# nihaomiao/WACV23_TSNet

Measured on AMD Instinct MI355X. Metric: retargeted frames/sec at bs=4, 256x256, n_source=3; max-abs delta vs ref, higher is better.
Workload: dtype f32 (convolutions: fp16 x 2 split of the scaled fp32 operands, 3 exact MFMA products, two-level fp32 accumulate; fp32-class accuracy); 1 GPU; TSNet(label_nc=2,n_blocks=0,n_downsampling=3,n_source=3) forward, fp32, B=4 per GPU, 256x256 (BASELINE.json configs[1]); global_batch=4, parallelism=replicas x1 (batch-sharded, weights broadcast once)

## Files before the change

### include/tsnet_abi.h

```cpp
#ifndef TSNET_ABI_H
#define TSNET_ABI_H

#include <stddef.h>
#include <stdint.h>

#ifdef __cplusplus
extern "C" {
#endif

#define TSNET_ABI_VERSION 5
#define TSNET_MAX_SOURCES 8

enum {
    TSNET_OK = 0,
    TSNET_ERR_ARG = -1,
    TSNET_ERR_WEIGHT = -2,
    TSNET_ERR_HIP = -3,
    TSNET_ERR_NOMEM = -4
};

typedef struct tsnet_engine* tsnet_handle;

typedef struct tsnet_cfg {
    int label_nc;
    int n_blocks;
    int n_downsampling;
    int n_source;
    int ngf;
    int enc_blocks;
    int addcoords;
    int pose_composite;
    float pose_mean[3];
    int height, width;
    int max_batch;
    int operand_mode;
} tsnet_cfg;

#define TSNET_NPROD_F16 16

int tsnet_abi_version(void);
int tsnet_create(const tsnet_cfg* cfg, tsnet_handle* out);
int tsnet_load_weights(tsnet_handle h, const char* name, const float* data, const int64_t* shape, int rank);
int tsnet_finalize(tsnet_handle h, void* stream);
void tsnet_destroy(tsnet_handle h);
const char* tsnet_last_error(tsnet_handle h);

int tsnet_num_params(tsnet_handle h);
int tsnet_param_info(tsnet_handle h, int index, const char** name, int64_t shape_out[4], int* rank);

int tsnet_packed_weights(tsnet_handle h, void** dev_ptr, size_t* bytes);

int tsnet_forward(tsnet_handle h,
                  const float* const* src_img, const float* const* src_lbl, const float* const* src_bbox,
                  const float* tar_lbl, const float* tar_bbox,
                  float* out_rgb, float* out_flow, int B, void* stream);

int tsnet_set_source_divisors(tsnet_handle h, const float* div, int n);

int tsnet_set_sources(tsnet_handle h, const float* const* src_img, const float* const* src_lbl,
                      const float* const* src_bbox, int B, void* stream);
int tsnet_forward_target(tsnet_handle h, const float* tar_lbl, const float* tar_bbox,
                         float* out_rgb, float* out_flow, int B, void* stream);

int tsnet_set_sources_shared(tsnet_handle h, const float* const* src_img, const float* const* src_lbl,
                             const float* const* src_bbox, void* stream);

int tsnet_bank_capacity(tsnet_handle h);
int tsnet_bank_put(tsnet_handle h, int first_slot, int count, const float* const* src_img, const float* const* src_lbl,
                   const float* const* src_bbox, const float* div, void* stream);
int tsnet_forward_bank(tsnet_handle h, const int* slots, int Kc, const float* tar_lbl, const float* tar_bbox,
                       float* out_rgb, float* out_flow, int B, void* stream);

int tsnet_forward_u8(tsnet_handle h, const uint8_t* const* src_img, const uint8_t* const* src_lbl, const uint8_t* const* src_bbox,
                     const uint8_t* tar_lbl, const uint8_t* tar_bbox, const float* mean_bgr,
                     float* out_rgb, float* out_flow, int B, void* stream);
int tsnet_set_sources_u8(tsnet_handle h, const uint8_t* const* src_img, const uint8_t* const* src_lbl, const uint8_t* const* src_bbox,
                         const float* mean_bgr, int B, int shared, void* stream);
int tsnet_forward_target_u8(tsnet_handle h, const uint8_t* tar_lbl, const uint8_t* tar_bbox,
                            float* out_rgb, float* out_flow, int B, void* stream);
int tsnet_bank_put_u8(tsnet_handle h, int first_slot, int count, const uint8_t* const* src_img, const uint8_t* const* src_lbl,
                      const uint8_t* const* src_bbox, const float* mean_bgr, const float* div, void* stream);
int tsnet_forward_bank_u8(tsnet_handle h, const int* slots, int Kc, const uint8_t* tar_lbl, const uint8_t* tar_bbox,
                          float* out_rgb, float* out_flow, int B, void* stream);

int tsnet_train_extras(tsnet_handle h, const float* const* src_img, const float* tar_img, int B,
                       float* warp_src_img, float* losses, void* stream);

int tsnet_stage_ptr(tsnet_handle h, const char* name, const float** dev_ptr, size_t* count);

double tsnet_forward_macs(tsnet_handle h, int B);

#define TSNET_TIMING_CLASSES 9
enum { TSNET_T_CONV = 0, TSNET_T_STATS = 1, TSNET_T_ELEMWISE = 2, TSNET_T_FLOW = 3, TSNET_T_WARP = 4,
       TSNET_T_PACK = 5, TSNET_T_UPSAMPLE = 6, TSNET_T_OTHER = 7,
       TSNET_T_CONV_RES = 8  };
int tsnet_timing_enable(tsnet_handle h, int on);
int tsnet_timing_read(tsnet_handle h, double ms_out[TSNET_TIMING_CLASSES], int64_t launches_out[TSNET_TIMING_CLASSES], int reset);

int tsnet_op_conv2d(const float* x, int N, int H, int W, int Cin,
                    const float* w_oihw, const float* bias, int Cout, int ksize, int stride, int pad, int pad_mode,
                    const float* in_alpha, const float* in_beta, int in_relu, float bound, int nprod, int kernel, int tile,
                    float* y, void* stream);
int tsnet_op_conv2d_cat(const float* x, const float* x2, int N, int H, int W, int C1, int C2, int x2_nmod,
                        const float* w_oihw, const float* bias, int Cout, int ksize, int stride, int pad, int pad_mode,
                        float bound, int nprod, float* y, void* stream);
int tsnet_op_head(const float* x, int N, int H, int W, int C, const float* in_alpha, const float* in_beta,
                  const float* w_oihw, const float* bias, int composite, const float* bg, float* y, void* stream);
int tsnet_op_instnorm_stats(const float* x, int N, int HW, int C, float* alpha, float* beta, void* stream);
int tsnet_op_norm_act(const float* x, const float* alpha, const float* beta, int relu, const float* resid,
                      int N, int HW, int C, float* y, void* stream);
int tsnet_op_upsample2x(const float* x, const float* alpha, const float* beta, int relu,
                        int N, int H, int W, int C, float* y, void* stream);
int tsnet_op_flow(const float* tar_fea, const float* src_fea, const float* tar_bbox, const float* src_bbox,
                  int B, int h, int w, int C, int H, int W, float* flow, void* stream);
int tsnet_op_flow_k(const float* tar_fea, const float* src_fea, const float* tar_bbox, const float* src_bbox,
                    int B, int K, int h, int w, int C, int H, int W, float* flow, int variant, int repeat, float* ms_out, void* stream);
int tsnet_flow_plan(int B, int h, int w, int C);
int tsnet_op_warp(const float* src_fea, const float* flow, int B, int h, int w, int C, float* out, void* stream);
int tsnet_op_warp_k(const float* src_fea, const float* flow, int B, int K, int h, int w, int C, float* out, int repeat, float* ms_out, void* stream);
int tsnet_op_warp_k_shared(const float* src_fea, const float* flow, int B, int K, int SB, int h, int w, int C, float* out, void* stream);
int tsnet_op_add_stats(const float* x, const float* add, int add_nmod, int x_sb, int N, int HW, int C,
                       float* y, float* alpha, float* beta, void* stream);
int tsnet_op_finalize_stats(const double* part, int N, int S, int C, int HW, float* alpha, float* beta, void* stream);
int tsnet_op_fuse_tail(const float* src_fea, const float* tar_fea, const float* y2, const float* alpha, const float* beta,
                       int B, int K, int SB, int P, int C1, float* zbar, void* stream);
int tsnet_op_flow_k_slots(const float* tar_fea, const float* src_fea, const float* tar_bbox, const float* src_bbox,
                          int B, int K, int h, int w, int C, int H, int W, float* flow, int variant, int repeat, float* ms_out,
                          const int* slots, int n_src, void* stream);
int tsnet_op_warp_k_slots(const float* src_fea, const float* flow, int B, int K, int h, int w, int C, float* out,
                          const int* slots, int n_src, void* stream);
int tsnet_op_add_stats_slots(const float* x, const float* add, int add_nmod, int N, int HW, int C,
                             float* y, float* alpha, float* beta, const int* slots, int n_src, void* stream);
int tsnet_op_fuse_tail_slots(const float* src_fea, const float* tar_fea, const float* y2, const float* alpha, const float* beta,
                             int B, int K, int P, int C1, float* zbar, const int* slots, int n_src, void* stream);
int tsnet_op_pack_input(const float* const* img, const float* const* lbl, int S, int B, int H, int W, int L, int nimg, int Cp, int coords,
                        const float* img_div, float* out, unsigned int* amax, void* stream);
int tsnet_op_pack_input_u8(const uint8_t* const* img, const uint8_t* const* lbl, const uint8_t* const* bbox, int S, int B, int H, int W, int L,
                           int nimg, int Cp, int coords, const float* img_div, const float* mean_bgr, float* out, float* bbox_out,
                           unsigned int* amax, void* stream);
int tsnet_op_upsample2x_st(const float* x, const float* alpha, const float* beta, int relu,
                           int N, int H, int W, int C, int x_bf16, int y_bf16, float* y, void* stream);
const char* tsnet_op_last_error(void);

int tsnet_frame_stats(const float* x, int B, int C, int HW, float div, float* mean, float* std_unbiased, void* stream);
int tsnet_demo_postprocess(const float* rec, int B, int H, int W, const float* gen_mean, const float* gen_std,
                           const float* ref_mean, const float* ref_std, const float* img_mean_over_255,
                           unsigned char* out_rgb, void* stream);

int tsnet_fit_face_curves(const double* keypoints, int F, double* curves);
int tsnet_raster_face(const double* keypoints, const double* curves, int F, int h, int w, int bw, unsigned char* edges, unsigned char* bbox, void* stream);
int tsnet_vl2ch(const float* labels, int B, int HW, int num_classes, float* out, void* stream);

int tsnet_face_adapt_stats(const double* kp, int F, double* stats);
int tsnet_face_adapt_apply(const double* stats, double* kp, int F);
int tsnet_smooth_keypoints(const double* in, int F, int P, double* out);

int tsnet_resize_label(const unsigned char* in, int F, int h, int w, int OH, int OW, const double* wts_rows, int lw_rows,
                       const double* wts_cols, int lw_cols, float* out, void* stream);
int tsnet_fit_pose_curves(const double* pts, int F, int flags, double* curves);
int tsnet_raster_pose(const double* pts, const double* curves, int F, int h, int w, int win_x0, int win_y0, int win_x1, int win_y1, int flags,
                      unsigned char* labels, void* stream);
int tsnet_label_bbox(const unsigned char* labels, int F, int h, int w, unsigned char* bbox, void* stream);
int tsnet_resize_pad(const unsigned char* in, int F, int h, int w, const int* ytab, const int* xtab, int oh, int ow,
                     int pad_top, int pad_left, int OH, int OW, int binarise, float* out, void* stream);

int tsnet_bench_conv(int N, int H, int W, int Cin, int Cout, int ksize, int stride, int pad, int pad_mode, int norm,
                     int variant, int iters, float* ms_out, void* stream);

void tsnet_debug_counters(int64_t out[4], int reset);

void tsnet_linspace(int n, float* out);
void tsnet_coord_table(int H, int W, float* out);

int tsnet_bicubic_taps(int n_in, int n_out);
int tsnet_bicubic_table(int n_in, int n_out, int* first, int* count, int* coef);
int tsnet_prepare_frames(const unsigned char* frames, int F, int h, int w, int x0, int y0, int x1, int y1,
                         const int* xfirst, const int* xcount, const int* xcoef, int xtaps,
                         const int* yfirst, const int* ycount, const int* ycoef, int ytaps,
                         int oh, int ow, int pad_top, int pad_left, int OH, int OW, const float* mean_bgr, float* out, void* stream);
int tsnet_prepare_frames_u8(const unsigned char* frames, int F, int h, int w, int x0, int y0, int x1, int y1,
                            const int* xfirst, const int* xcount, const int* xcoef, int xtaps,
                            const int* yfirst, const int* ycount, const int* ycoef, int ytaps,
                            int oh, int ow, int pad_top, int pad_left, int OH, int OW, unsigned char* out, void* stream);

int tsnet_paste_frames(const unsigned char* gen, const unsigned char* mask, int F, int GH, int GW, int sx0, int sy0, int sx1, int sy1,
// ... 26 lines not shown
```

### wacv23_tsnet_amd/_lib.py

```python
from __future__ import annotations

import ctypes as C
import os

import torch

_HERE = os.path.dirname(os.path.abspath(__file__))
LIB_PATH = os.path.join(_HERE, "lib", "libtsnet_hip.so")
MAX_SOURCES = 8
TIMING_CLASSES = 9
TIMING_NAMES = ("conv", "stats", "elementwise", "flow", "warp", "pack", "upsample", "other", "conv_res")

ABI_SYMBOLS = (
    "tsnet_abi_version", "tsnet_create", "tsnet_load_weights", "tsnet_finalize", "tsnet_destroy",
    "tsnet_last_error", "tsnet_num_params", "tsnet_param_info", "tsnet_packed_weights",
    "tsnet_forward", "tsnet_set_source_divisors", "tsnet_set_sources", "tsnet_set_sources_shared", "tsnet_forward_target", "tsnet_train_extras", "tsnet_stage_ptr",
    "tsnet_forward_macs", "tsnet_timing_enable", "tsnet_timing_read",
    "tsnet_op_conv2d", "tsnet_op_conv2d_cat", "tsnet_op_head", "tsnet_op_instnorm_stats", "tsnet_op_norm_act", "tsnet_op_upsample2x",
    "tsnet_op_flow", "tsnet_op_flow_k", "tsnet_flow_plan", "tsnet_op_warp", "tsnet_op_warp_k", "tsnet_op_warp_k_shared", "tsnet_op_add_stats", "tsnet_op_finalize_stats", "tsnet_op_fuse_tail", "tsnet_op_pack_input", "tsnet_op_upsample2x_st", "tsnet_op_last_error", "tsnet_frame_stats", "tsnet_demo_postprocess", "tsnet_fit_face_curves", "tsnet_raster_face", "tsnet_vl2ch", "tsnet_fit_pose_curves", "tsnet_raster_pose", "tsnet_label_bbox", "tsnet_resize_pad", "tsnet_resize_label", "tsnet_bench_conv", "tsnet_debug_counters", "tsnet_linspace", "tsnet_coord_table",
    "tsnet_bicubic_taps", "tsnet_bicubic_table", "tsnet_prepare_frames",
    "tsnet_face_adapt_stats", "tsnet_face_adapt_apply", "tsnet_smooth_keypoints",
    "tsnet_bank_capacity", "tsnet_bank_put", "tsnet_forward_bank",
    "tsnet_op_flow_k_slots", "tsnet_op_warp_k_slots", "tsnet_op_add_stats_slots", "tsnet_op_fuse_tail_slots",
    "tsnet_forward_u8", "tsnet_set_sources_u8", "tsnet_forward_target_u8", "tsnet_bank_put_u8", "tsnet_forward_bank_u8",
    "tsnet_op_pack_input_u8", "tsnet_prepare_frames_u8",
    "tsnet_paste_frames",
    "tsnet_prepare_frames_boxes", "tsnet_prepare_frames_boxes_u8", "tsnet_paste_frames_boxes",
    "tsnet_face_labels_boxes", "tsnet_face_labels_boxes_u8",
)


class TsnetCfg(C.Structure):
    _fields_ = [
        ("label_nc", C.c_int), ("n_blocks", C.c_int), ("n_downsampling", C.c_int), ("n_source", C.c_int),
        ("ngf", C.c_int), ("enc_blocks", C.c_int), ("addcoords", C.c_int), ("pose_composite", C.c_int),
        ("pose_mean", C.c_float * 3), ("height", C.c_int), ("width", C.c_int), ("max_batch", C.c_int), ("operand_mode", C.c_int),
    ]


_fp = C.POINTER(C.c_float)
_vp = C.c_void_p


def bind(lib: C.CDLL) -> C.CDLL:
    lib.tsnet_abi_version.restype = C.c_int
    lib.tsnet_create.argtypes = [C.POINTER(TsnetCfg), C.POINTER(_vp)]
    lib.tsnet_load_weights.argtypes = [_vp, C.c_char_p, _vp, C.POINTER(C.c_int64), C.c_int]
    lib.tsnet_finalize.argtypes = [_vp, _vp]
    lib.tsnet_destroy.argtypes = [_vp]
    lib.tsnet_destroy.restype = None
    lib.tsnet_last_error.argtypes = [_vp]
    lib.tsnet_last_error.restype = C.c_char_p
    lib.tsnet_num_params.argtypes = [_vp]
    lib.tsnet_param_info.argtypes = [_vp, C.c_int, C.POINTER(C.c_char_p), C.POINTER(C.c_int64), C.POINTER(C.c_int)]
    lib.tsnet_packed_weights.argtypes = [_vp, C.POINTER(_vp), C.POINTER(C.c_size_t)]
    pp = C.POINTER(_vp)
    lib.tsnet_forward.argtypes = [_vp, pp, pp, pp, _vp, _vp, _vp, _vp, C.c_int, _vp]
    lib.tsnet_set_source_divisors.argtypes = [_vp, _fp, C.c_int]
    lib.tsnet_set_sources.argtypes = [_vp, pp, pp, pp, C.c_int, _vp]
    if hasattr(lib, "tsnet_set_sources_shared"):
        lib.tsnet_set_sources_shared.argtypes = [_vp, pp, pp, pp, _vp]
    lib.tsnet_forward_target.argtypes = [_vp, _vp, _vp, _vp, _vp, C.c_int, _vp]
    lib.tsnet_train_extras.argtypes = [_vp, pp, _vp, C.c_int, _vp, _vp, _vp]
    lib.tsnet_stage_ptr.argtypes = [_vp, C.c_char_p, C.POINTER(_vp), C.POINTER(C.c_size_t)]
    lib.tsnet_forward_macs.argtypes = [_vp, C.c_int]
    lib.tsnet_forward_macs.restype = C.c_double
    lib.tsnet_timing_enable.argtypes = [_vp, C.c_int]
    lib.tsnet_timing_read.argtypes = [_vp, C.POINTER(C.c_double), C.POINTER(C.c_int64), C.c_int]
    lib.tsnet_op_conv2d.argtypes = [_vp, C.c_int, C.c_int, C.c_int, C.c_int, _vp, _vp, C.c_int, C.c_int, C.c_int,
                                    C.c_int, C.c_int, _vp, _vp, C.c_int, C.c_float, C.c_int, C.c_int, C.c_int, _vp, _vp]
    lib.tsnet_op_conv2d_cat.argtypes = [_vp, _vp] + [C.c_int] * 6 + [_vp, _vp] + [C.c_int] * 5 + [C.c_float, C.c_int, _vp, _vp]
    lib.tsnet_op_head.argtypes = [_vp, C.c_int, C.c_int, C.c_int, C.c_int, _vp, _vp, _vp, _vp, C.c_int, _fp, _vp, _vp]
    lib.tsnet_op_instnorm_stats.argtypes = [_vp, C.c_int, C.c_int, C.c_int, _vp, _vp, _vp]
    lib.tsnet_op_norm_act.argtypes = [_vp, _vp, _vp, C.c_int, _vp, C.c_int, C.c_int, C.c_int, _vp, _vp]
    lib.tsnet_op_upsample2x.argtypes = [_vp, _vp, _vp, C.c_int, C.c_int, C.c_int, C.c_int, C.c_int, _vp, _vp]
    lib.tsnet_resize_label.argtypes = [_vp, C.c_int, C.c_int, C.c_int, C.c_int, C.c_int, _vp, C.c_int, _vp, C.c_int, _vp, _vp]
    lib.tsnet_op_flow.argtypes = [_vp, _vp, _vp, _vp, C.c_int, C.c_int, C.c_int, C.c_int, C.c_int, C.c_int, _vp, _vp]
    lib.tsnet_op_flow_k.argtypes = [_vp, _vp, _vp, _vp] + [C.c_int] * 7 + [_vp, C.c_int, C.c_int, _fp, _vp]
    lib.tsnet_flow_plan.argtypes = [C.c_int] * 4
    lib.tsnet_op_warp.argtypes = [_vp, _vp, C.c_int, C.c_int, C.c_int, C.c_int, _vp, _vp]
    if hasattr(lib, "tsnet_op_warp_k"):
        lib.tsnet_op_warp_k.argtypes = [_vp, _vp] + [C.c_int] * 5 + [_vp, C.c_int, _fp, _vp]
    if hasattr(lib, "tsnet_op_fuse_tail"):
        lib.tsnet_op_warp_k_shared.argtypes = [_vp, _vp] + [C.c_int] * 6 + [_vp, _vp]
        lib.tsnet_op_add_stats.argtypes = [_vp, _vp] + [C.c_int] * 5 + [_vp, _vp, _vp, _vp]
        lib.tsnet_op_finalize_stats.argtypes = [_vp] + [C.c_int] * 4 + [_vp, _vp, _vp]
        lib.tsnet_op_fuse_tail.argtypes = [_vp] * 5 + [C.c_int] * 5 + [_vp, _vp]
        lib.tsnet_op_pack_input.argtypes = [pp, pp] + [C.c_int] * 8 + [_fp, _vp, _vp, _vp]
        lib.tsnet_op_upsample2x_st.argtypes = [_vp, _vp, _vp] + [C.c_int] * 7 + [_vp, _vp]
    lib.tsnet_op_last_error.restype = C.c_char_p
    lib.tsnet_frame_stats.argtypes = [_vp, C.c_int, C.c_int, C.c_int, C.c_float, _vp, _vp, _vp]
    lib.tsnet_demo_postprocess.argtypes = [_vp, C.c_int, C.c_int, C.c_int, _vp, _vp, _vp, _vp, _fp, _vp, _vp]
    lib.tsnet_fit_face_curves.argtypes = [_vp, C.c_int, _vp]
    lib.tsnet_fit_pose_curves.argtypes = [_vp, C.c_int, C.c_int, _vp]
    lib.tsnet_raster_face.argtypes = [_vp, _vp, C.c_int, C.c_int, C.c_int, C.c_int, _vp, _vp, _vp]
    lib.tsnet_vl2ch.argtypes = [_vp, C.c_int, C.c_int, C.c_int, _vp, _vp]
    lib.tsnet_raster_pose.argtypes = [_vp, _vp] + [C.c_int] * 8 + [_vp, _vp]
    lib.tsnet_label_bbox.argtypes = [_vp, C.c_int, C.c_int, C.c_int, _vp, _vp]
    lib.tsnet_resize_pad.argtypes = [_vp, C.c_int, C.c_int, C.c_int, _vp, _vp] + [C.c_int] * 7 + [_vp, _vp]
    lib.tsnet_bench_conv.argtypes = [C.c_int] * 12 + [_fp, _vp]
    lib.tsnet_debug_counters.argtypes = [C.POINTER(C.c_int64), C.c_int]
    lib.tsnet_debug_counters.restype = None
    lib.tsnet_linspace.argtypes = [C.c_int, _fp]
    lib.tsnet_linspace.restype = None
    lib.tsnet_coord_table.argtypes = [C.c_int, C.c_int, _fp]
    lib.tsnet_coord_table.restype = None
    if hasattr(lib, "tsnet_prepare_frames"):
        lib.tsnet_bicubic_taps.argtypes = [C.c_int, C.c_int]
        lib.tsnet_bicubic_table.argtypes = [C.c_int, C.c_int, _vp, _vp, _vp]
        lib.tsnet_prepare_frames.argtypes = [_vp] + [C.c_int] * 7 + [_vp, _vp, _vp, C.c_int, _vp, _vp, _vp, C.c_int] + [C.c_int] * 6 + [_fp, _vp, _vp]
    if hasattr(lib, "tsnet_face_adapt_stats"):
        lib.tsnet_face_adapt_stats.argtypes = [_vp, C.c_int, _vp]
        lib.tsnet_face_adapt_apply.argtypes = [_vp, _vp, C.c_int]
        lib.tsnet_smooth_keypoints.argtypes = [_vp, C.c_int, C.c_int, _vp]
    if hasattr(lib, "tsnet_forward_bank"):
        _ip = C.POINTER(C.c_int)
        lib.tsnet_bank_capacity.argtypes = [_vp]
        lib.tsnet_bank_put.argtypes = [_vp, C.c_int, C.c_int, pp, pp, pp, _fp, _vp]
        lib.tsnet_forward_bank.argtypes = [_vp, _ip, C.c_int, _vp, _vp, _vp, _vp, C.c_int, _vp]
        lib.tsnet_op_flow_k_slots.argtypes = [_vp, _vp, _vp, _vp] + [C.c_int] * 7 + [_vp, C.c_int, C.c_int, _fp, _ip, C.c_int, _vp]
        lib.tsnet_op_warp_k_slots.argtypes = [_vp, _vp] + [C.c_int] * 5 + [_vp, _ip, C.c_int, _vp]
        lib.tsnet_op_add_stats_slots.argtypes = [_vp, _vp] + [C.c_int] * 4 + [_vp, _vp, _vp, _ip, C.c_int, _vp]
        lib.tsnet_op_fuse_tail_slots.argtypes = [_vp] * 5 + [C.c_int] * 4 + [_vp, _ip, C.c_int, _vp]
    if hasattr(lib, "tsnet_forward_u8"):
        _ip = C.POINTER(C.c_int)
        lib.tsnet_forward_u8.argtypes = [_vp, pp, pp, pp, _vp, _vp, _fp, _vp, _vp, C.c_int, _vp]
        lib.tsnet_set_sources_u8.argtypes = [_vp, pp, pp, pp, _fp, C.c_int, C.c_int, _vp]
        lib.tsnet_forward_target_u8.argtypes = [_vp, _vp, _vp, _vp, _vp, C.c_int, _vp]
        lib.tsnet_bank_put_u8.argtypes = [_vp, C.c_int, C.c_int, pp, pp, pp, _fp, _fp, _vp]
        lib.tsnet_forward_bank_u8.argtypes = [_vp, _ip, C.c_int, _vp, _vp, _vp, _vp, C.c_int, _vp]
        lib.tsnet_op_pack_input_u8.argtypes = [pp, pp, pp] + [C.c_int] * 8 + [_fp, _fp, _vp, _vp, _vp, _vp]
        lib.tsnet_prepare_frames_u8.argtypes = [_vp] + [C.c_int] * 7 + [_vp, _vp, _vp, C.c_int, _vp, _vp, _vp, C.c_int] + [C.c_int] * 6 + [_vp, _vp]
    if hasattr(lib, "tsnet_paste_frames"):
        lib.tsnet_paste_frames.argtypes = [_vp, _vp] + [C.c_int] * 7 + [_vp, _vp, _vp, C.c_int, _vp, _vp, _vp, C.c_int] + [_vp] + [C.c_int] * 6 + [_vp]
    if hasattr(lib, "tsnet_paste_frames_boxes"):
        lib.tsnet_prepare_frames_boxes.argtypes = [_vp] + [C.c_int] * 3 + [_vp, _vp, _vp, C.c_int] + [C.c_int] * 6 + [_fp, _vp, _vp]
        lib.tsnet_prepare_frames_boxes_u8.argtypes = [_vp] + [C.c_int] * 3 + [_vp, _vp, _vp, C.c_int] + [C.c_int] * 6 + [_vp, _vp]
        lib.tsnet_paste_frames_boxes.argtypes = [_vp, _vp] + [C.c_int] * 7 + [_vp, _vp, _vp, C.c_int] + [_vp, C.c_int, C.c_int, _vp]
    if hasattr(lib, "tsnet_face_labels_boxes"):
        for fn in (lib.tsnet_face_labels_boxes, lib.tsnet_face_labels_boxes_u8):
            fn.argtypes = [_vp, _vp, C.c_int, _vp, _vp, _vp, C.c_int, C.c_int, _vp, C.c_longlong, C.c_int, C.c_int, _vp, _vp, _vp]
    return lib


_cached = None


def load_tools() -> C.CDLL:
    from . import build as _b
    if not os.path.exists(_b.OUT_TOOLS):
        raise RuntimeError(f"{_b.OUT_TOOLS} is missing: run `python -m wacv23_tsnet_amd.build --tools`")
    return bind(C.CDLL(_b.OUT_TOOLS))


def load() -> C.CDLL:
    global _cached
    if _cached is not None:
        return _cached
    if not os.path.exists(LIB_PATH):
        raise RuntimeError(
            f"{LIB_PATH} is missing: the HIP extension is not built. Run "
            "`python -c 'import __graft_entry__ as g; g.build()'` (needs hipcc). "
            "There is no CPU fallback for the TS-Net forward path.")
    try:
        _cached = bind(C.CDLL(LIB_PATH))
    except OSError as e:
        raise RuntimeError(f"failed to load {LIB_PATH}: {e}") from e
    if _cached.tsnet_abi_version() != 5:
        raise RuntimeError("libtsnet_hip.so ABI version mismatch; rebuild")
    return _cached
```

### wacv23_tsnet_amd/csrc/conv_common.hpp

```cpp
#pragma once
#include <hip/hip_runtime.h>

namespace tsnet {

typedef float f32x16 __attribute__((ext_vector_type(16)));
struct alignas(16) F4 { float v[4]; };

constexpr unsigned kOOB = 0x80000000u;
constexpr int kPatchCols = 32;
constexpr int kPatchRows = 4;

constexpr int kNprodF16 = 16;
constexpr bool one_product(int nprod) { return nprod == 1 || nprod == kNprodF16; }

#ifndef TSNET_BUF_LOAD16
typedef __amdgpu_buffer_rsrc_t tsnet_brsrc_t;
__device__ __forceinline__ tsnet_brsrc_t tsnet_make_brsrc(const void* p, unsigned bytes) {
    return __builtin_amdgcn_make_buffer_rsrc(const_cast<void*>(p), 0, (int)bytes, 0x00020000);
}
#define TSNET_BUF_LOAD16(rsrc, voff, soff) __builtin_bit_cast(F4, __builtin_amdgcn_raw_buffer_load_b128((rsrc), (int)(voff), (int)(soff), 0))
#endif
#ifndef TSNET_BUF_LOAD8
struct alignas(8) F2 { float v[2]; };
#define TSNET_BUF_LOAD8(rsrc, voff, soff) __builtin_bit_cast(F2, __builtin_amdgcn_raw_buffer_load_b64((rsrc), (int)(voff), (int)(soff), 0))
// ... 142 lines not shown
    int xcd_gn;
    float* fin_alpha; float* fin_beta; int* fin_counter; int fin_S; float fin_eps;
    unsigned* amax_out;
    int x_bf16, y_bf16;
    int w1_chunk, w1_tab2;
};

__device__ __forceinline__ void bf16x8_widen(const F4& p, F4 (&o)[2]) {
#pragma unroll
    for (int e = 0; e < 4; ++e) {
        const unsigned w = __builtin_bit_cast(unsigned, p.v[e]);
        o[e >> 1].v[(e & 1) * 2] = __builtin_bit_cast(float, w << 16);
        o[e >> 1].v[(e & 1) * 2 + 1] = __builtin_bit_cast(float, w & 0xFFFF0000u);
    }
}

__device__ __forceinline__ void load_x_octet(const tsnet_brsrc_t& rs, bool xb16, unsigned voff, unsigned soff, F4 (&o)[2]) {
    if (xb16) {
        const F4 p = TSNET_BUF_LOAD16(rs, voff >> 1, soff >> 1);
        bf16x8_widen(p, o);
    } else {
        o[0] = TSNET_BUF_LOAD16(rs, voff, soff);
        o[1] = TSNET_BUF_LOAD16(rs, voff, soff + 16u);
    }
}

__device__ __forceinline__ void h2_device_scale(const unsigned* amax, float add, float& scale, float& unscale) {
    const float bound = __builtin_bit_cast(float, __hip_atomic_load(amax, __ATOMIC_RELAXED, __HIP_MEMORY_SCOPE_AGENT)) + add;
    int e = 0;
    (void)frexpf(bound, &e);
    int sa = 15 - e;
    sa = sa > 24 ? 24 : (sa < -24 ? -24 : sa);
    scale = ldexpf(1.0f, sa);
    unscale = ldexpf(1.0f, -sa);
}

__device__ __forceinline__ void split_h2(float v, unsigned& hi, unsigned& lo) {
    const _Float16 h = (_Float16)v;
    const _Float16 l = (_Float16)(v - (float)h);
    hi = (unsigned)__builtin_bit_cast(unsigned short, h);
    lo = (unsigned)__builtin_bit_cast(unsigned short, l);
}

__device__ __forceinline__ void split_h2_octet(const F4& x0, const F4& x1, F4& H, F4& L) {
    unsigned hw[4], lw[4];
    TSNET_SPLIT_2PAIRS(x0.v[0], x0.v[1], x0.v[2], x0.v[3], hw[0], lw[0], hw[1], lw[1]);
    TSNET_SPLIT_2PAIRS(x1.v[0], x1.v[1], x1.v[2], x1.v[3], hw[2], lw[2], hw[3], lw[3]);
#pragma unroll
    for (int e = 0; e < 4; ++e) { H.v[e] = __builtin_bit_cast(float, hw[e]); L.v[e] = __builtin_bit_cast(float, lw[e]); }
}

template <bool F16 = false>
__device__ __forceinline__ void one_plane_octet(const F4& x0, const F4& x1, F4& H) {
    unsigned hw[4];
#pragma unroll
    for (int e = 0; e < 2; ++e) {
        hw[e] = cvt_pk_one<F16>(x0.v[2 * e], x0.v[2 * e + 1]);
        hw[2 + e] = cvt_pk_one<F16>(x1.v[2 * e], x1.v[2 * e + 1]);
    }
#pragma unroll
    for (int e = 0; e < 4; ++e) H.v[e] = __builtin_bit_cast(float, hw[e]);
}

template <bool AFFINE, bool KEEP = true>
__device__ __forceinline__ void transform_octet(const F4 (&sx)[2], const float* ta, int Cin, float in_scale, float relu_floor, float keep, F4 (&t)[2]) {
    if (AFFINE) {
#pragma unroll
        for (int q = 0; q < 2; ++q) {
            const F4 al = *reinterpret_cast<const F4*>(ta + q * 4), be = *reinterpret_cast<const F4*>(ta + Cin + q * 4);
#pragma unroll
            for (int e = 0; e < 4; ++e) {
                const float v = __builtin_fmaxf(__builtin_fmaf(sx[q].v[e], al.v[e], be.v[e]), relu_floor);
                t[q].v[e] = KEEP ? v * keep : v;
            }
        }
    } else {
#pragma unroll
        for (int q = 0; q < 2; ++q)
#pragma unroll
            for (int e = 0; e < 4; ++e) t[q].v[e] = __builtin_fmaxf(sx[q].v[e] * in_scale, relu_floor);
    }
}

template <int BN, int WARPS_M, int WARPS_N, int MT, int NTL, int STAT_WAVE = 0, typename MOf>
__device__ __forceinline__ void conv_epilogue(const ConvArgs& a, f32x16 (&tot)[MT][NTL], unsigned char* smem_raw, int tid, int wave, int n0,
                                              size_t stat_tile, MOf m_of, const bool active = true) {
    constexpr int WM = MT * 32, WN = NTL * 32;
    const int lane = tid & 63, li = lane & 31, lh = lane >> 5;
    const int wm0 = (wave / WARPS_N) * WM, wn0 = (wave % WARPS_N) * WN;
    const int hw = a.Ho * a.Wo;
    double csum[NTL], csq[NTL];
#pragma unroll
    for (int j = 0; j < NTL; ++j) { csum[j] = 0.0; csq[j] = 0.0; }
    float vmax = 0.f;
#pragma unroll
    for (int i = 0; i < MT; ++i) {
#pragma unroll
        for (int j = 0; j < NTL; ++j) {
            const int n = n0 + wn0 + j * 32 + li;
            const bool nok = n < a.Cout;
            const float bv = (a.bias && nok) ? a.bias[n] : 0.f;
#pragma unroll
            for (int r = 0; r < 16; ++r) {
                const int m = m_of(wm0 + i * 32 + (r & 3) + 8 * (r >> 2) + 4 * lh);
                const bool mok = active && m >= 0;
                float v = tot[i][j][r] + bv;
                if (a.addend && nok && mok) {
                    const int img = m / hw;
                    v += a.addend[((size_t)(img % a.add_nmod) * hw + (m - img * hw)) * a.Cout + n];
                }
                tot[i][j][r] = v;
                if (a.stat_part && mok) { csum[j] += (double)v; csq[j] += (double)v * (double)v; }
                if (nok && mok) vmax = __builtin_fmaxf(vmax, __builtin_fabsf(v));
            }
        }
    }
    if (a.amax_out) tsnet_publish_amax(a.amax_out + stat_tile / (size_t)a.tpi, vmax);
    if (a.stat_part) {
        __syncthreads();
        double* red = reinterpret_cast<double*>(smem_raw);
#pragma unroll
        for (int j = 0; j < NTL; ++j) {
            const double s2 = csum[j] + __shfl_xor(csum[j], 32);
            const double q2 = csq[j] + __shfl_xor(csq[j], 32);
            if (lh == 0 && active) {
                double* o = red + ((size_t)(wave / WARPS_N) * BN + wn0 + j * 32 + li) * 2;
                o[0] = s2; o[1] = q2;
            }
        }
        __syncthreads();
        const int stid = tid - 64 * STAT_WAVE;
        if (stid >= 0 && stid < BN && n0 + stid < a.Cout) {
            double s = 0.0, q = 0.0;
#pragma unroll
            for (int wmi = 0; wmi < WARPS_M; ++wmi) { s += red[((size_t)wmi * BN + stid) * 2]; q += red[((size_t)wmi * BN + stid) * 2 + 1]; }
            double* o = a.stat_part + (stat_tile * a.Cout + n0 + stid) * 2;
            if (a.fin_counter) {
                __hip_atomic_store(o, s, __ATOMIC_RELAXED, __HIP_MEMORY_SCOPE_AGENT);
                __hip_atomic_store(o + 1, q, __ATOMIC_RELAXED, __HIP_MEMORY_SCOPE_AGENT);
            } else {
                o[0] = s; o[1] = q;
            }
        }
        if (a.fin_counter) {
            const int S = a.fin_S;
            const int img = (int)(stat_tile / (size_t)S);
            const int ntn = (a.Npad + 31) / 32;
            int* counter = a.fin_counter + (size_t)img * ntn + n0 / 32;
            const bool mine = stid >= 0 && stid < BN && n0 + stid < a.Cout;
            auto fold = [&](const double* p0, int cnt, size_t step, double& sm, double& sq) __attribute__((always_inline)) {
                double gs[4] = {0, 0, 0, 0}, gq[4] = {0, 0, 0, 0};
                for (int t0 = 0; t0 < cnt; t0 += 8) {
                    double v[8], w[8];
#pragma unroll
                    for (int u = 0; u < 8; ++u) {
                        const double* p = p0 + (size_t)(t0 + u < cnt ? t0 + u : cnt - 1) * step;
                        v[u] = __hip_atomic_load(p, __ATOMIC_RELAXED, __HIP_MEMORY_SCOPE_AGENT);
                        w[u] = __hip_atomic_load(p + 1, __ATOMIC_RELAXED, __HIP_MEMORY_SCOPE_AGENT);
                    }
#pragma unroll
                    for (int u = 0; u < 8; ++u) {
                        const bool in = t0 + u < cnt;
                        gs[u & 3] += in ? v[u] : 0.0;
                        gq[u & 3] += in ? w[u] : 0.0;
                    }
                }
// ... 65 lines not shown
```

### wacv23_tsnet_amd/csrc/conv_h2.hpp

```cpp
#pragma once
#include "conv_common.hpp"

namespace tsnet {

template <int PR, int BN, int WARPS_M, int WARPS_N, int NPROD, bool AFFINE, int HABL = 0, int OPT = 0>
__device__ __forceinline__ void h2_tile(const ConvArgs& a, unsigned char* smem_raw, const int tile_m, const int n0) {
    constexpr int BM = PR * kPatchCols;
    constexpr int NW = WARPS_M * WARPS_N;
    static_assert(NW == 4, "four waves: patch blocks are dealt w, w+4");
    static_assert(one_product(NPROD) || NPROD == 3 || NPROD == 4, "one (a bf16 or an fp16 plane), three or four products");
    constexpr bool ONEP = one_product(NPROD), F16P = NPROD == kNprodF16;
    constexpr int NPL = ONEP ? 1 : 2;
    constexpr bool DEEP = (OPT & 8) != 0;
    constexpr int BD = DEEP ? 9 : ((OPT & 32) ? 6 : 3);
    constexpr bool ONE_LEVEL = ONEP;
    constexpr bool ZPAD_KEEP = (OPT & 1) != 0;
    constexpr int CH = (OPT & 2) ? 1 : ((OPT & 4) ? 4 : 2);
    constexpr int KG = (OPT & 16) ? 2 : 1;
    constexpr int WM = BM / WARPS_M, WN = BN / WARPS_N;
    constexpr int MT = WM / 32, NTL = WN / 32;
    static_assert(WARPS_M * MT == PR, "a wave covers MT whole patch rows");
    constexpr int NRW = MT + 2;
    constexpr int PC = kPatchCols + 2, PP = (PR + 2) * PC;
    constexpr int PBLK = (PP + 31) / 32;
    static_assert(PBLK <= 8, "two staging rounds");
    constexpr int REGION = PBLK * 512;
    constexpr int PLANE_P = 2 * REGION, PATCH_BYTES = NPL * PLANE_P;
    constexpr int OFF_SINK = 2 * 2 * PLANE_P;
    constexpr int GROUP_BYTES = OFF_SINK + 2048;
    constexpr int OFF_TAB = KG * GROUP_BYTES;

    const int tid = threadIdx.x;
    const int lane = tid & 63;
    const int wave_all = TSNET_UNIFORM(tid >> 6);
    const int kg = KG == 1 ? 0 : wave_all >> 2;
    const int wave = KG == 1 ? wave_all : (wave_all & 3);
    unsigned char* const gbase = smem_raw + kg * GROUP_BYTES;
    const int wrow = wave / WARPS_N;
    const int wn0 = (wave % WARPS_N) * WN;
    const int li = lane & 31, lh = lane >> 5;

    const int tcols = a.Wo / kPatchCols, tper = (a.Ho / PR) * tcols;
    const int img = tile_m / tper, tin = tile_m - img * tper;
    const int oy0 = (tin / tcols) * PR, ox0 = (tin % tcols) * kPatchCols;
    const int ncc = a.Cin >> 4;
    float in_scale = a.in_scale, in_unscale = a.in_unscale;
    if (NPROD != 1 && a.in_amax) h2_device_scale(a.in_amax + img, a.in_bound_add, in_scale, in_unscale);

    const size_t planew = (size_t)((a.nchunks + 1) / 2 * 2) * a.Npad * 16;
    const bool xb16 = NPROD == 1 && a.x_bf16;
    const tsnet_brsrc_t rsx = tsnet_make_brsrc(a.x, (unsigned)((size_t)a.N * a.H * a.W * a.Cin * (xb16 ? 2 : 4)));
    tsnet_brsrc_t rsw[NPL];
#pragma unroll
    for (int p = 0; p < NPL; ++p) rsw[p] = tsnet_make_brsrc(a.w + p * planew, (unsigned)(planew * 2));

    const int oct = lane >> 5;
    unsigned vP[2];
    float vM[2];
#pragma unroll
    for (int r = 0; r < 2; ++r) {
        const int pp = (wave + 4 * r) * 32 + (lane & 31);
        const int pr = pp / PC, pc = pp - pr * PC;
        int iy = oy0 - 1 + pr, ix = ox0 - 1 + pc;
        bool ok = pp < PP;
        if (a.reflect) {
            iy = iy < 0 ? -iy : iy;
            iy = iy >= a.H ? 2 * (a.H - 1) - iy : iy;
            ix = ix < 0 ? -ix : ix;
            ix = ix >= a.W ? 2 * (a.W - 1) - ix : ix;
        } else {
            ok = ok && iy >= 0 && iy < a.H && ix >= 0 && ix < a.W;
        }
        const int pix = iy * a.W + ix;
        vP[r] = ok ? (unsigned)(((img * a.H * a.W + pix) * a.Cin + oct * 8) * 4) : kOOB;
        vM[r] = ok ? 1.f : 0.f;
    }
    float* tab = reinterpret_cast<float*>(smem_raw + OFF_TAB);
    if (AFFINE) {
        for (int c = tid; c < a.Cin; c += 256 * KG) {
            tab[c] = a.in_alpha[(size_t)img * a.Cin + c] * in_scale;
            tab[a.Cin + c] = a.in_beta[(size_t)img * a.Cin + c] * in_scale;
        }
        __syncthreads();
    }
    const float relu_floor = a.in_relu ? 0.f : -__builtin_inff();
    auto slab_of = [&](int lc) __attribute__((always_inline)) { return lc * KG + kg; };
    F4 sx[2][2];
    auto stage_load_x = [&](int cn, int r) __attribute__((always_inline)) {
        if (NPROD == 1) load_x_octet(rsx, xb16, vP[r], (unsigned)(slab_of(cn) * 64), sx[r]);
        else {
#pragma unroll
            for (int q = 0; q < 2; ++q) sx[r][q] = TSNET_BUF_LOAD16(rsx, vP[r], (unsigned)(slab_of(cn) * 64 + q * 16));
        }
    };
    auto stage_store = [&](int cn, int par, int r) __attribute__((always_inline)) {
        const int b = wave + 4 * r;
        F4 t[2];
        const float* ta = tab + (slab_of(cn) < ncc ? slab_of(cn) * 16 : 0) + oct * 8;
        transform_octet<AFFINE, ZPAD_KEEP>(sx[r], ta, a.Cin, in_scale, relu_floor, vM[r], t);
        unsigned char* dst = gbase + (b < PBLK ? par * PATCH_BYTES + oct * REGION + b * 512 : OFF_SINK + oct * 512) + (lane & 31) * 16;
        F4 Hh, Ll;
        if (ONEP) {
            one_plane_octet<F16P>(t[0], t[1], Hh);
            *reinterpret_cast<F4*>(dst) = Hh;
        } else {
            split_h2_octet(t[0], t[1], Hh, Ll);
            *reinterpret_cast<F4*>(dst) = Hh;
            *reinterpret_cast<F4*>(dst + (b < PBLK ? PLANE_P : 1024)) = Ll;
        }
    };

    const unsigned vB = (unsigned)((wn0 + li) * 32 + (lh ^ ((li >> 3) & 1)) * 16);
    constexpr bool DB = MT > 2;
    static_assert(!DB || NRW == 6, "the double-buffered form fetches two rows of the next tap column per step");
    F4 ar[DB ? 2 : 1][NRW][NPL], bf[BD][NPL][NTL];
    auto tap_of = [](int s) __attribute__((always_inline)) { return (s % 3) * 3 + s / 3; };
    const int wB = a.Npad * 32, wT = ncc * wB;
    int wsl = slab_of(0) * wB + n0 * 32;
    auto load_b = [&](int set, int dslab, int s) __attribute__((always_inline)) {
        const int soff = wsl + dslab * KG * wB + tap_of(s) * wT;
#pragma unroll
        for (int p = 0; p < NPL; ++p)
#pragma unroll
            for (int j = 0; j < NTL; ++j) bf[set][p][j] = TSNET_BUF_LOAD16(rsw[p], vB + j * 1024u, (unsigned)soff);
    };
    const unsigned char* abase = gbase + lh * REGION + (wrow * MT * PC + li) * 16;
    auto load_row = [&](int r, int par, int kx) __attribute__((always_inline)) {
        const unsigned char* pbase = abase + par * PATCH_BYTES;
#pragma unroll
        for (int p = 0; p < NPL; ++p) ar[DB ? (kx & 1) : 0][r][p] = *reinterpret_cast<const F4*>(pbase + p * PLANE_P + (r * PC + kx) * 16);
    };

    f32x16 acc[MT][NTL], tot[MT][NTL];
#pragma unroll
    for (int i = 0; i < MT; ++i)
#pragma unroll
        for (int j = 0; j < NTL; ++j)
#pragma unroll
            for (int r = 0; r < 16; ++r) { acc[i][j][r] = 0.f; tot[i][j][r] = 0.f; }

    auto product = [&](int kx, int ky, int sb, int pa, int pb, bool fresh) __attribute__((always_inline)) {
#pragma unroll
        for (int i = 0; i < MT; ++i)
#pragma unroll
            for (int j = 0; j < NTL; ++j) {
                f32x16 c = acc[i][j];
                if (fresh) {
#pragma unroll
                    for (int r = 0; r < 16; ++r) c[r] = 0.f;
                }
                if (NPROD == 1) acc[i][j] = TSNET_MFMA_BF16(ar[DB ? (kx & 1) : 0][i + ky][pa], bf[sb][pb][j], c);
                else acc[i][j] = TSNET_MFMA_F16(ar[DB ? (kx & 1) : 0][i + ky][pa], bf[sb][pb][j], c);
            }
    };
    auto step = [&](int cc, int par, int s, bool first, bool last) __attribute__((always_inline)) {
        const int kx = s / 3, ky = s % 3;
        const bool fresh = !ONE_LEVEL && first;
        const int s2 = (s + BD - 1) % 9;
        if (!(HABL & 2)) load_b((par * 9 + s + BD - 1) % BD, s + BD - 1 >= 9 ? 1 : 0, s2);
        if (!(HABL & 4)) {
            if (DB) {
                if (kx < 2) { load_row(2 * ky, par, kx + 1); load_row(2 * ky + 1, par, kx + 1); }
            } else {
                if (ky < 2) load_row(ky + MT, par, kx);
                if (kx < 2 && ky == 1) {
#pragma unroll
                    for (int r = 0; r + 1 < MT; ++r) load_row(r, par, kx + 1);
                }
                if (kx < 2 && ky == 2) load_row(MT - 1, par, kx + 1);
            }
        }
        if (s == 0 && !(HABL & 1)) stage_load_x(cc + 1, 0);
        if (s == (DEEP ? 1 : 3) && !(HABL & 1)) stage_load_x(cc + 1, 1);
        const int SB = (par * 9 + s) % BD;
        if (ONEP) {
            product(kx, ky, SB, 0, 0, fresh);
        } else {
            if (NPROD == 4) product(kx, ky, SB, NPL - 1, NPL - 1, fresh);
            product(kx, ky, SB, NPL - 1, 0, fresh && NPROD == 3);
            product(kx, ky, SB, 0, NPL - 1, false);
            product(kx, ky, SB, 0, 0, false);
        }
        if (s == (DEEP ? 5 : 2) && !(HABL & 1)) stage_store(cc + 1, par ^ 1, 0);
        if (s == (DEEP ? 7 : 5) && !(HABL & 1)) stage_store(cc + 1, par ^ 1, 1);
        __builtin_amdgcn_sched_barrier(0);
        if (!ONE_LEVEL && last && !(HABL & 8)) {
#pragma unroll
            for (int i = 0; i < MT; ++i)
#pragma unroll
                for (int j = 0; j < NTL; ++j)
#pragma unroll
                    for (int r = 0; r < 16; ++r) tot[i][j][r] += acc[i][j][r];
        }
    };
    auto slab = [&](int cc, int par, bool open, bool close) __attribute__((always_inline)) {
        if (!(HABL & 16)) __syncthreads();
        if ((!(HABL & 4) || cc == 0) && !(DB && (HABL & 8) && cc > 0)) {
#pragma unroll
            for (int r = 0; r < (DB ? NRW : MT); ++r) load_row(r, par, 0);
        }
#pragma unroll
        for (int s = 0; s < 9; ++s) step(cc, par, s, open && s == 0, close && s == 8);
        wsl += KG * wB;
    };

    stage_load_x(0, 0); stage_load_x(0, 1);
#pragma unroll
    for (int i = 0; i < BD - 1; ++i) load_b(i, 0, i);
    stage_store(0, 0, 0); stage_store(0, 0, 1);
    if (HABL & 2) load_b(2, 0, 2);
    if (HABL & 4) {
        __syncthreads();
#pragma unroll
        for (int r = 0; r < NRW; ++r) load_row(r, 0, 0);
    }
    const int nloc = ncc / KG;
    int cc = 0;
    if (CH == 4) {
        for (; cc + 4 <= nloc; cc += 4) { slab(cc, 0, true, false); slab(cc + 1, 1, false, false); slab(cc + 2, 0, false, false); slab(cc + 3, 1, false, true); }
    }
    if (CH == 1) {
        for (; cc + 2 <= nloc; cc += 2) { slab(cc, 0, true, true); slab(cc + 1, 1, true, true); }
    } else {
        for (; cc + 2 <= nloc; cc += 2) { slab(cc, 0, true, false); slab(cc + 1, 1, false, true); }
    }
    if (cc < nloc) slab(cc, 0, true, true);
    if (ONE_LEVEL) {
#pragma unroll
        for (int i = 0; i < MT; ++i)
#pragma unroll
            for (int j = 0; j < NTL; ++j) tot[i][j] = acc[i][j];
    }
    if (KG == 2) {
        __syncthreads();
        float* fold = reinterpret_cast<float*>(smem_raw) + (size_t)wave * (MT * NTL * 16 * 64) + lane;
        if (kg == 1) {
#pragma unroll
            for (int i = 0; i < MT; ++i)
#pragma unroll
                for (int j = 0; j < NTL; ++j)
#pragma unroll
                    for (int r = 0; r < 16; ++r) fold[((i * NTL + j) * 16 + r) * 64] = tot[i][j][r];
        }
        __syncthreads();
        if (kg == 0) {
#pragma unroll
            for (int i = 0; i < MT; ++i)
#pragma unroll
                for (int j = 0; j < NTL; ++j)
#pragma unroll
                    for (int r = 0; r < 16; ++r) tot[i][j][r] += fold[((i * NTL + j) * 16 + r) * 64];
        }
    }

    const float unscale = a.w_unscale ? in_unscale * a.w_unscale[0] : in_unscale;
#pragma unroll
    for (int i = 0; i < MT; ++i)
#pragma unroll
        for (int j = 0; j < NTL; ++j)
#pragma unroll
            for (int r = 0; r < 16; ++r) tot[i][j][r] *= unscale;
    const int m_img = img * a.Ho * a.Wo;
    conv_epilogue<BN, WARPS_M, WARPS_N, MT, NTL>(a, tot, smem_raw, tid, wave, n0, (size_t)img * tper + tin,
                                                 [&](int l) { return m_img + (oy0 + (l >> 5)) * a.Wo + ox0 + (l & 31); }, kg == 0);
}

constexpr int h2_lds_bytes(int PR, int Cin, int KG = 1) { return KG * (2 * 2 * 2 * (((PR + 2) * (kPatchCols + 2) + 31) / 32) * 512 + 2048) + 2 * Cin * 4; }

template <int PR, int BN, int WARPS_M, int WARPS_N, int NPROD, int OPT>
constexpr int h2_wgs_per_cu() { return (OPT & 16) ? 1 : ((BN / WARPS_N) * (PR / WARPS_M) * ((OPT & 8) ? 2 : 1) <= (one_product(NPROD) ? 128 : 64) ? ((OPT & 64) ? 4 : 3) : 2); }

template <int PR, int BN, int WARPS_M, int WARPS_N, int NPROD, bool AFFINE, int HABL = 0, int OPT = 0>
__global__ __launch_bounds__((OPT & 16) ? 512 : 256, (h2_wgs_per_cu<PR, BN, WARPS_M, WARPS_N, NPROD, OPT>()))
void conv_h2_kernel(ConvArgs a) {
    HIP_DYNAMIC_SHARED(__attribute__((aligned(16))) unsigned char, smem_raw)
    int tile_m, tile_n;
    tile_of_block(blockIdx.x, a.tiles_m, a.tiles_n, a.xcd_gn, tile_m, tile_n);
    h2_tile<PR, BN, WARPS_M, WARPS_N, NPROD, AFFINE, HABL, OPT>(a, smem_raw, tile_m, tile_n * BN);
}

template <int NPROD>
__device__ __forceinline__ void h2s_tile(const ConvArgs& a, unsigned char* smem_raw, const int tile_m, const int n0) {
    constexpr int BN = 64, WARPS_M = 2, WARPS_N = 2, MT = 2, NTL = 1;
    constexpr bool ONEP = one_product(NPROD), F16P = NPROD == kNprodF16;
    constexpr int NPL = ONEP ? 1 : 2;
    constexpr int PC = kPatchCols + 6, PR = kPatchRows + 6, PP = PR * PC;
    constexpr int PLANE_S = 384 * 16;
    static_assert(one_product(NPROD) || NPROD == 3, "one (a bf16 or an fp16 plane) or three products");

    const int tid = threadIdx.x;
    const int lane = tid & 63;
    const int wave = TSNET_UNIFORM(tid >> 6);
    const int wrow = wave / WARPS_N;
    const int wn0 = (wave % WARPS_N) * 32;
    const int li = lane & 31, lh = lane >> 5;

    const int tcols = a.Wo / kPatchCols, tper = (a.Ho / kPatchRows) * tcols;
    const int img = tile_m / tper, tin = tile_m - img * tper;
    const int oy0 = (tin / tcols) * kPatchRows, ox0 = (tin % tcols) * kPatchCols;
    float in_scale = a.in_scale, in_unscale = a.in_unscale;
    if (NPROD != 1 && a.in_amax) h2_device_scale(a.in_amax + img, a.in_bound_add, in_scale, in_unscale);

    const size_t planew = (size_t)((a.nchunks + 1) / 2 * 2) * a.Npad * 16;
    const tsnet_brsrc_t rsx = tsnet_make_brsrc(a.x, (unsigned)((size_t)a.N * a.H * a.W * 8 * 4));
    tsnet_brsrc_t rsw[NPL];
#pragma unroll
    for (int p = 0; p < NPL; ++p) rsw[p] = tsnet_make_brsrc(a.w + p * planew, (unsigned)(planew * 2));

    const unsigned vB = (unsigned)((wn0 + li) * 32 + (lh ^ ((li >> 3) & 1)) * 16);
    F4 af[2][NPL][MT], bf[3][NPL];
    auto load_b = [&](int set, int kc) __attribute__((always_inline)) {
#pragma unroll
        for (int p = 0; p < NPL; ++p) bf[set][p] = TSNET_BUF_LOAD16(rsw[p], vB, (unsigned)((kc * a.Npad + n0) * 32));
    };
    load_b(0, 0);
    load_b(1, 1);

#pragma unroll
    for (int r = 0; r < 2; ++r) {
        const int pp = tid + r * 256;
        const int pr = pp / PC, pc = pp - pr * PC;
        int iy = oy0 - 3 + pr, ix = ox0 - 3 + pc;
        iy = iy < 0 ? -iy : iy;
        iy = iy >= a.H ? 2 * (a.H - 1) - iy : iy;
        ix = ix < 0 ? -ix : ix;
        ix = ix >= a.W ? 2 * (a.W - 1) - ix : ix;
        const unsigned v = pp < PP ? (unsigned)((((img * a.H + iy) * a.W) + ix) * 32) : kOOB;
        F4 x0 = TSNET_BUF_LOAD16(rsx, v, 0u), x1 = TSNET_BUF_LOAD16(rsx, v, 16u);
#pragma unroll
        for (int e = 0; e < 4; ++e) { x0.v[e] *= in_scale; x1.v[e] *= in_scale; }
        if (pp < 384) {
            F4 Hh, Ll;
            if (ONEP) {
                one_plane_octet<F16P>(x0, x1, Hh);
                *reinterpret_cast<F4*>(smem_raw + pp * 16) = Hh;
            } else {
                split_h2_octet(x0, x1, Hh, Ll);
                *reinterpret_cast<F4*>(smem_raw + pp * 16) = Hh;
                *reinterpret_cast<F4*>(smem_raw + PLANE_S + pp * 16) = Ll;
            }
        }
    }
    __syncthreads();

    const int base = (wrow * MT * PC + li) * 16;
    struct StepTab { int off[25], delta[25]; };
    static constexpr StepTab kStep = [] {
        StepTab t{};
        for (int st = 0; st < 25; ++st) {
            const int t0 = 2 * st, ky = t0 / 7, kx = t0 - ky * 7;
            t.off[st] = (ky * PC + kx) * 16;
            t.delta[st] = st >= 24 ? 0 : (kx == 6 ? (PC - 6) * 16 : 16);
        }
        return t;
    }();
    auto load_a = [&](int set, int st) __attribute__((always_inline)) {
        const unsigned char* b = smem_raw + base + kStep.off[st] + lh * kStep.delta[st];
#pragma unroll
        for (int i = 0; i < MT; ++i)
#pragma unroll
            for (int p = 0; p < NPL; ++p) af[set][p][i] = *reinterpret_cast<const F4*>(b + p * PLANE_S + i * PC * 16);
// ... 296 lines not shown
```

### wacv23_tsnet_amd/csrc/conv_h2_launch.cpp

```cpp
#include <map>
#include <mutex>
#include <stdexcept>
#include <string>
#include <utility>

#include "conv_h2.hpp"
#include "kernels.hpp"

namespace tsnet {

void ensure_dynamic_lds(const void* kernel, size_t bytes) {
    if (bytes <= 48 * 1024) return;
    static std::mutex mu;
    static std::map<std::pair<const void*, int>, size_t> done;
    int dev = 0;
    (void)hipGetDevice(&dev);
    std::lock_guard<std::mutex> lk(mu);
    size_t& have = done[std::make_pair(kernel, dev)];
    if (have >= bytes) return;
    const hipError_t e = hipFuncSetAttribute(kernel, hipFuncAttributeMaxDynamicSharedMemorySize, (int)bytes);
    if (e != hipSuccess) throw std::runtime_error(std::string("hipFuncSetAttribute(MaxDynamicSharedMemorySize) failed: ") + hipGetErrorString(e));
    have = bytes;
}

namespace {

template <int PR, int BN, int WM, int WN, int NPROD, bool AFFINE, int HABL, int OPT>
void go_h2_k(const ConvArgs& a, size_t lds, int threads, hipStream_t s) {
    launch_tiles(conv_h2_kernel<PR, BN, WM, WN, NPROD, AFFINE, HABL, OPT>, threads, lds, a, s);
}

template <int PR, int BN, int WM, int WN, int NPROD, int HABL = 0, int OPT = 0>
void go_h2(const ConvArgs& a, hipStream_t s) {
    constexpr int KG = (OPT & 16) ? 2 : 1;
    static_assert((OPT & 1) == 0, "bit 0 is chosen here");
    const size_t lds = (size_t)h2_lds_bytes(PR, a.Cin, KG);
    if (!a.in_alpha) go_h2_k<PR, BN, WM, WN, NPROD, false, HABL, OPT>(a, lds, 256 * KG, s);
    else if (a.reflect) go_h2_k<PR, BN, WM, WN, NPROD, true, HABL, OPT>(a, lds, 256 * KG, s);
    else go_h2_k<PR, BN, WM, WN, NPROD, true, HABL, OPT | 1>(a, lds, 256 * KG, s);
}

template <int NPROD>
void go_h2_shape(const ConvArgs& a, const ConvPlan& p, hipStream_t s) {
    const int pr = p.rows, bn = p.width;
    if (pr == 4 && bn == 32) return go_h2<4, 32, 4, 1, NPROD>(a, s);
    if (pr == 4 && bn == 64) return go_h2<4, 64, 2, 2, NPROD>(a, s);
    if (pr == 4 && bn == 128 && !p.side_by_side) return go_h2<4, 128, 2, 2, NPROD>(a, s);
    if (pr == 2 && bn == 128) return go_h2<2, 128, 1, 4, NPROD>(a, s);
    if constexpr (one_product(NPROD)) {
        if (pr == 4 && bn == 128) return go_h2<4, 128, 1, 4, NPROD>(a, s);
    }
    plan_not_built(p, NPROD);
}

template <int BN, int NWV, int NPROD, int PR = kPatchRows, bool DEEP = false>
void go_h2d(const ConvArgs& a, hipStream_t s) {
    launch_tiles(a.in_alpha ? conv_h2d_kernel<BN, NWV, NPROD, true, PR, DEEP> : conv_h2d_kernel<BN, NWV, NPROD, false, PR, DEEP>, 64 * NWV, (size_t)h2d_lds_bytes(PR) + (size_t)2 * a.Cin * 4, a, s);
}

}

void launch_conv_h2(const ConvArgs& a, const ConvPlan& p, int nprod, int abl, int opt, hipStream_t s) {
    const int pr = p.rows, bn = p.width;
    if (p.sched == ConvSched::TwoGroups) {
        if (pr == 4 && bn == 32) return nprod == 3 ? go_h2<4, 32, 4, 1, 3, 0, 24>(a, s) : (nprod == kNprodF16 ? go_h2<4, 32, 4, 1, kNprodF16, 0, 24>(a, s) : go_h2<4, 32, 4, 1, 1, 0, 24>(a, s));
        if (pr == 4 && bn == 64) return nprod == 3 ? go_h2<4, 64, 2, 2, 3, 0, 24>(a, s) : (nprod == kNprodF16 ? go_h2<4, 64, 2, 2, kNprodF16, 0, 24>(a, s) : go_h2<4, 64, 2, 2, 1, 0, 24>(a, s));
        plan_not_built(p, nprod);
    }
    if (abl || opt) {
#ifdef TSNET_TOOLS
        if (nprod == 1) {
#define TSNET_H2_VAR1(A_) if (pr == 4 && bn == 128 && !p.side_by_side && abl == A_ && opt == 0) { go_h2<4, 128, 2, 2, 1, A_, 0>(a, s); return; }
            TSNET_H2_VAR1(1) TSNET_H2_VAR1(2) TSNET_H2_VAR1(4) TSNET_H2_VAR1(3) TSNET_H2_VAR1(7) TSNET_H2_VAR1(16)
#undef TSNET_H2_VAR1
#define TSNET_H2_VAR1S(A_) if (pr == 4 && bn == 128 && p.side_by_side && abl == A_ && opt == 0) { go_h2<4, 128, 1, 4, 1, A_, 0>(a, s); return; }
            TSNET_H2_VAR1S(1) TSNET_H2_VAR1S(2) TSNET_H2_VAR1S(4) TSNET_H2_VAR1S(3) TSNET_H2_VAR1S(7) TSNET_H2_VAR1S(16) TSNET_H2_VAR1S(8)
#undef TSNET_H2_VAR1S
            throw std::invalid_argument("conv(h2): this bf16 experiment variant is not instantiated");
        }
        if (nprod != 3) throw std::invalid_argument("conv(h2): experiment variants are built for one or three products");
#define TSNET_H2_VAR(PR_, BN_, WM_, WN_, A_, O_) if (pr == PR_ && bn == BN_ && abl == A_ && opt == O_) { go_h2<PR_, BN_, WM_, WN_, 3, A_, O_>(a, s); return; }
        TSNET_H2_VAR(4, 64, 2, 2, 0, 2) TSNET_H2_VAR(4, 64, 2, 2, 0, 4) TSNET_H2_VAR(4, 64, 2, 2, 0, 8) TSNET_H2_VAR(4, 64, 2, 2, 0, 16)
        TSNET_H2_VAR(4, 128, 2, 2, 0, 2) TSNET_H2_VAR(4, 128, 2, 2, 0, 4) TSNET_H2_VAR(4, 128, 2, 2, 0, 16) TSNET_H2_VAR(4, 32, 4, 1, 0, 8)
        TSNET_H2_VAR(4, 64, 2, 2, 0, 32) TSNET_H2_VAR(4, 64, 2, 2, 0, 64) TSNET_H2_VAR(4, 64, 2, 2, 0, 36) TSNET_H2_VAR(2, 128, 1, 4, 0, 32)
        TSNET_H2_VAR(4, 64, 2, 2, 1, 0) TSNET_H2_VAR(4, 64, 2, 2, 2, 0) TSNET_H2_VAR(4, 64, 2, 2, 4, 0) TSNET_H2_VAR(4, 64, 2, 2, 7, 0)
        TSNET_H2_VAR(4, 64, 2, 2, 8, 0) TSNET_H2_VAR(4, 64, 2, 2, 16, 0) TSNET_H2_VAR(4, 64, 2, 2, 15, 0) TSNET_H2_VAR(4, 64, 2, 2, 31, 0)
        TSNET_H2_VAR(2, 128, 1, 4, 1, 0) TSNET_H2_VAR(2, 128, 1, 4, 2, 0) TSNET_H2_VAR(2, 128, 1, 4, 7, 0)
#undef TSNET_H2_VAR
        throw std::invalid_argument("conv(h2): this experiment variant is not instantiated");
#else
        throw std::invalid_argument("conv(h2): experiment / ablation variants are only built into the tools library");
#endif
    }
    if (nprod == 3) go_h2_shape<3>(a, p, s);
    else if (nprod == 1) go_h2_shape<1>(a, p, s);
    else if (nprod == kNprodF16) go_h2_shape<kNprodF16>(a, p, s);
    else if (pr == 4 && bn == 64) go_h2<4, 64, 2, 2, 4>(a, s);
    else if (pr == 4 && bn == 128) go_h2<4, 128, 2, 2, 4>(a, s);
    else plan_not_built(p, nprod);
}

void launch_conv_h2s(const ConvArgs& a, int nprod, hipStream_t s) {
    if (nprod == 3) hipLaunchKernelGGL((conv_h2s_kernel<3>), dim3(a.tiles_m * a.tiles_n), dim3(256), kH2sLds, s, a);
    else if (nprod == kNprodF16) hipLaunchKernelGGL((conv_h2s_kernel<kNprodF16>), dim3(a.tiles_m * a.tiles_n), dim3(256), kH2sLds, s, a);
    else hipLaunchKernelGGL((conv_h2s_kernel<1>), dim3(a.tiles_m * a.tiles_n), dim3(256), kH2sLds, s, a);
}

void launch_conv_h2d(const ConvArgs& a, const ConvPlan& p, int nprod, hipStream_t s) {
    const int pr = p.rows, bn = p.width;
    if (p.sched == ConvSched::Deep) {
        if (pr == 2 && bn == 128 && nprod == 3) return go_h2d<128, 4, 3, 2, true>(a, s);
    } else {
        if (pr == 4 && bn == 64) return nprod == 3 ? go_h2d<64, 4, 3>(a, s) : (nprod == kNprodF16 ? go_h2d<64, 4, kNprodF16>(a, s) : go_h2d<64, 4, 1>(a, s));
        if (pr == 4 && bn == 128) return nprod == 3 ? go_h2d<128, 8, 3>(a, s) : (nprod == kNprodF16 ? go_h2d<128, 8, kNprodF16>(a, s) : go_h2d<128, 8, 1>(a, s));
        if (pr == 2 && bn == 128) return nprod == 3 ? go_h2d<128, 4, 3, 2>(a, s) : (nprod == kNprodF16 ? go_h2d<128, 4, kNprodF16, 2>(a, s) : go_h2d<128, 4, 1, 2>(a, s));
    }
    plan_not_built(p, nprod);
}

}
```

### wacv23_tsnet_amd/csrc/conv_plan.hpp

```cpp
#pragma once
#include <cstddef>
#include <stdexcept>
#include <string>

namespace tsnet {

constexpr int kPlanTileRows = 4, kPlanTileCols = 32;
constexpr size_t kFinCounterInts = 65536;
constexpr int kFinMaxTiles = 32;

enum class ConvFamily { H2R, G64, H2, H2S, H2S32, H2D, W1 };
enum class ConvKernel { Own = 0, General = 1, Patch = 2 };
enum class ConvSched { Plain = 0, Deep = 1, TwoGroups = 2 };

struct ConvShape {
    int ks = 1, stride = 1, pad = 0, reflect = 0;
    int cin = 0;
    int cout = 0, npad = 0, kpad = 0;
    int form = 0;
    int N = 0, H = 0, W = 0;
    int csplit = 0;
    int x2_nmod = 1;
    bool transform = false;
    int nprod = 3;
    bool f16 = false;
    bool fin_counter = false;
    int ho() const { return (H + 2 * pad - ks) / stride + 1; }
    int wo() const { return (W + 2 * pad - ks) / stride + 1; }
};

struct ConvRequest {
    ConvKernel kernel = ConvKernel::Own;
    int rows = 0;
    int width = 0;
    bool alt = false;
    ConvSched sched = ConvSched::Plain;
    int chunk = 0;
    int chunk_cap = 3;
    int abl = 0, opt = 0;
    int xcd_gn = -1;
};

struct ConvPlan {
    ConvFamily family = ConvFamily::H2R;
    int rows = 0;
    int width = 0;
    bool side_by_side = false;
    ConvSched sched = ConvSched::Plain;
    int w1_chunk = 1, w1_tab2 = 0;
    int xcd_gn = 0;
    int tpi = 0, tiles_m = 0, tiles_n = 0;
    bool fin = false;
};

inline ConvRequest decode_tile_code(int kernel, int tile) {
    ConvRequest r;
    if (kernel == 3) {
        if (tile < 0 || tile > 3) throw std::invalid_argument("conv: the Winograd form takes 0 to 3 tiles per workgroup");
        r.chunk = tile;
        return r;
    }
    if (kernel < 0 || kernel > 2) throw std::invalid_argument("conv: kernel must be 0 (the layer's own), 1 (general), 2 (patch) or 3 (Winograd form)");
    r.kernel = static_cast<ConvKernel>(kernel);
    switch (tile) {
        case 0: break;
        case 32: case 64: case 128: r.width = tile; break;
        case 2128: r.rows = 2; r.width = 128; break;
        case 3064: case 3128: r.alt = true; r.width = tile - 3000; break;
        case 12128: r.rows = 2; r.width = 128; r.sched = ConvSched::Deep; break;
        case 20032: case 20064: r.rows = 4; r.width = tile - 20000; r.sched = ConvSched::TwoGroups; break;
        default: throw std::invalid_argument("conv: unknown tile code " + std::to_string(tile));
    }
    return r;
}

struct BenchVariant { ConvRequest req; int nprod = 3, form = 0; bool cold = false; };
inline BenchVariant decode_bench_variant(int variant) {
    const int v = variant < 0 ? 0 : variant;
    BenchVariant b;
    b.form = (v & 32768) ? 1 : 0;
    b.req = decode_tile_code(b.form ? 3 : ((v & 4096) ? 1 : ((v & 16384) ? 2 : 0)), v & 4095);
    b.nprod = (v & 8192) ? 1 : 3;
    b.cold = (v & (1 << 21)) != 0;
    b.req.abl = (v >> 16) & 31;
    b.req.opt = ((v >> 24) & 15) | ((v & (1 << 23)) ? 16 : 0) | ((v & (1 << 22)) ? 32 : 0);
    if (!b.req.abl && b.req.opt == (8 | 16)) { b.req.sched = ConvSched::TwoGroups; b.req.opt = 0; }
    const int gx = (v >> 28) & 7;
    if (gx > 5) throw std::invalid_argument("bench_conv: XCD grid code 0 to 5");
    b.req.xcd_gn = gx == 0 ? -1 : (gx == 1 ? 0 : 1 << (gx - 2));
    return b;
}

struct HeadRequest { bool composite = false; int rows = 0; };
inline HeadRequest decode_head_code(int code) {
    if (code < 0 || (code & 0xFE)) throw std::invalid_argument("head: composite is bit 0, the tile rows bits 8 and up");
    HeadRequest r;
    r.composite = code & 1;
    r.rows = code >> 8;
    if (r.rows != 0 && r.rows != 8 && r.rows != 16 && r.rows != 32) throw std::invalid_argument("head: tile rows 8, 16 or 32");
    return r;
}

constexpr size_t w1_lds_bytes_host(int Cin, int tables) {
    return 3 * (size_t)(2 * (4 * 2 * 2 * (96 * 16 + 64) + 16)) + (size_t)tables * 2 * ((Cin + 31) / 32 * 32) * 4;
}
inline bool w1_eligible(int ks, int stride, int pad, int cin, int H, int W) {
    return ks == 3 && stride == 1 && pad == 1 && cin >= 16 && (cin & 15) == 0 && H >= 4 && W >= 32 && H % kPlanTileRows == 0 && W % kPlanTileCols == 0 &&
           w1_lds_bytes_host(cin, 1) + 256 <= 160 * 1024;
}

inline void validate_conv(const ConvShape& s) {
    auto refuse = [](const char* why) { throw std::invalid_argument(why); };
    if (s.ks != 1 && s.ks != 3 && s.ks != 7) refuse("conv: kernel size must be 1, 3 or 7");
    if (s.cin != 8 && (s.cin < 16 || (s.cin & 15))) refuse("conv: input channels must be 8 or a multiple of 16 (pad with zeros)");
    if (s.stride < 1 || s.pad < 0) refuse("conv: the stride must be positive, the padding not negative");
    if (s.N < 1 || s.H < 1 || s.W < 1 || s.H + 2 * s.pad < s.ks || s.W + 2 * s.pad < s.ks || s.cout < 1) refuse("conv: empty tensor");
    if (s.reflect && (s.pad >= s.H || s.pad >= s.W)) refuse("conv: reflection pad needs pad < input size");
    if (s.csplit && ((s.csplit & 15) || s.csplit < 0 || s.csplit >= s.cin)) refuse("conv: channel split must be a multiple of 16 inside the channel range");
    const double px = (double)s.H * s.W * 4, c1 = s.csplit ? s.csplit : s.cin;
    if (s.N * px * c1 >= 2147483648.0 || s.x2_nmod * px * (s.cin - c1) >= 2147483648.0 || (double)s.N * s.ho() * s.wo() * s.cout >= 2147483647.0 ||
        (double)s.kpad * s.npad * 2 >= 2147483648.0)
        refuse("conv: tensor too large for 32-bit buffer offsets");
    if ((size_t)2 * s.cin * 4 > 32 * 1024) refuse("conv: too many input channels for the transform table");
}

inline ConvFamily conv_class(const ConvShape& s, int rows, bool eligible_only) {
    const int Ho = s.ho(), Wo = s.wo();
    const bool onep = s.nprod == 1;
    const bool s1 = s.ks == 3 && s.stride == 1 && s.pad == 1 && s.cin >= 16 && (s.cin & 15) == 0 && s.H >= 2 && s.W >= 2;
    if (s.csplit || Ho <= 0 || Wo <= 0 || Wo % kPlanTileCols) return ConvFamily::H2R;
    const bool s2 = s.ks == 3 && s.stride == 2 && s.pad == 1 && !s.reflect && s.cin >= (eligible_only ? 16 : 128) && (s.cin & 15) == 0 && s.H == 2 * Ho && s.W == 2 * Wo;
    if (rows == 2 && Ho % 2 == 0) {
        if (s1) return ConvFamily::H2;
        if (s2) return ConvFamily::H2D;
    }
    if (Ho % kPlanTileRows) return ConvFamily::H2R;
    if (s1) return ConvFamily::H2;
    if (s.ks == 7 && s.stride == 1 && s.pad == 3 && s.reflect && s.cin == 8 && !s.transform && s.H >= 4 && s.W >= 4) return ConvFamily::H2S;
    if (s.ks == 7 && s.stride == 1 && s.pad == 3 && s.reflect && s.cin == 32 && !s.transform && s.H >= 4 && s.W >= 4) return ConvFamily::H2S32;
    if (s2 && (eligible_only || !onep)) return ConvFamily::H2D;
    return ConvFamily::H2R;
}

inline bool wide_pays(const ConvShape& s, long tm, double gain, int cus) {
    const double c64 = (double)((tm * ((s.cout + 63) / 64) + cus - 1) / cus) * 64.0;
    const double c128 = (double)((tm * ((s.cout + 127) / 128) + cus - 1) / cus) * 128.0 / gain;
    return s.npad % 128 == 0 && s.cout > 64 && c128 < c64;
}

inline int xcd_grid(const ConvShape& s, int requested, int tiles_m, int tiles_n, const char* who) {
    int gn = requested < 0 ? (((double)s.kpad * s.npad * 4 > 16e6) ? 4 : 0) : requested;
    if (gn && ((gn != 1 && gn != 2 && gn != 4 && gn != 8) || tiles_n % gn || tiles_m % (8 / gn))) {
        if (requested >= 0) throw std::invalid_argument(std::string(who) + ": the XCD grid does not divide the tile matrix");
        gn = 0;
    }
    return gn;
}

inline void plan_w1_chunk(const ConvShape& s, const ConvRequest& r, int cus, ConvPlan& p) {
    const int n = p.tiles_m * p.tiles_n, npp = ((s.cin >> 4) + 1) / 2;
    const int rows = p.xcd_gn ? p.tiles_m / (8 / p.xcd_gn) : (p.tiles_m % 8 ? 0 : p.tiles_m / 8);
    const bool tab2 = !s.transform || w1_lds_bytes_host(s.cin, 2) + 256 <= 160 * 1024;
    auto fits = [&](int cc) { return cc == 1 || (s.nprod != 1 && npp >= 4 && rows > 0 && rows % cc == 0 && (tab2 || p.tpi % cc == 0)); };
    int cc = 1;
    if (r.chunk) {
        if (!fits(r.chunk)) throw std::invalid_argument("conv(w1): this chunk size does not fit the layer");
        cc = r.chunk;
    } else {
        for (int t : {3, 2}) if (fits(t) && n % (cus * t) == 0) { cc = t; break; }
        if (cc > r.chunk_cap) cc = 1;
    }
    p.w1_chunk = cc; p.w1_tab2 = (s.transform && tab2 && cc > 1) ? 1 : 0;
}

inline ConvPlan plan_conv(const ConvShape& s, const ConvRequest& r, int cus) {
    validate_conv(s);
    const bool onep = s.nprod == 1;
    const int Ho = s.ho(), hw = Ho * s.wo();
    ConvPlan p;
    if (s.form == 1) {
        if (s.csplit || !w1_eligible(s.ks, s.stride, s.pad, s.cin, s.H, s.W))
            throw std::invalid_argument("conv(w1): the layer is packed in the Winograd form, which needs a single source and whole 4 x 32 tiles");
        if (s.f16) throw std::invalid_argument("conv(w1): the Winograd form is not built for fp16 operands (one fp16 plane); its one-product form takes bf16 operands");
        p.family = ConvFamily::W1;
    } else if (r.kernel == ConvKernel::General) {
        p.family = ConvFamily::H2R;
    } else {
        p.family = conv_class(s, r.rows == 2 ? 2 : kPlanTileRows, r.kernel == ConvKernel::Patch);
        if (r.kernel == ConvKernel::Patch && p.family == ConvFamily::H2R) throw std::invalid_argument("conv: this layer / frame size has no patch kernel");
    }
    if (s.nprod != 1 && s.nprod != 3 && (s.nprod != 4 || p.family != ConvFamily::H2))
        throw std::invalid_argument("conv: 1 (bf16 operands), 16 (fp16 operands) or 3 products; four on the 3x3 / stride-1 patch kernel's plain 4x64 and 4x128 tiles");
    if (s.f16 && s.nprod != 1) throw std::invalid_argument("conv: fp16 operands (one fp16 plane) run one product");
    auto set_tiles = [&](int rows_per_tile_m, int bn) {
        p.tpi = (hw + rows_per_tile_m - 1) / rows_per_tile_m;
        p.tiles_m = s.N * p.tpi; p.tiles_n = (s.cout + bn - 1) / bn;
        p.fin = s.fin_counter && p.tpi <= kFinMaxTiles && (size_t)s.N * ((s.npad + 31) / 32) <= kFinCounterInts;
    };
    switch (p.family) {
    case ConvFamily::W1:
        if (r.opt || r.sched != ConvSched::Plain) throw std::invalid_argument("conv(w1): no experiment variants");
        p.rows = kPlanTileRows; p.width = 64;
        set_tiles(kPlanTileRows * kPlanTileCols, 64);
        p.xcd_gn = xcd_grid(s, r.xcd_gn, p.tiles_m, p.tiles_n, "conv(w1)");
        plan_w1_chunk(s, r, cus, p);
        break;
    case ConvFamily::H2: {
        int pr = r.rows ? r.rows : kPlanTileRows, bn = r.width;
        if (bn == 0) {
            const long tm = (long)s.N * (hw / 128);
            bn = wide_pays(s, tm, s.transform ? 1.03 : 1.10, cus) ? 128 : 64;
            if (onep && s.npad % 128 == 0 && s.cout > 64 && tm * ((s.cout + 127) / 128) >= cus) bn = 128;
        }
        p.side_by_side = r.alt || (!r.width && onep && pr == 4 && bn == 128);
        if (p.side_by_side && (!onep || bn != 128 || pr != 4)) throw std::invalid_argument("conv(h2): the 1 x 4 wave grid is the bf16 4 x 128 tile's (and its fp16-operand twin's: one product)");
        if (!(pr == 4 && (bn == 32 || bn == 64 || bn == 128)) && !(pr == 2 && bn == 128)) throw std::invalid_argument("conv(h2): tile must be 4x32, 4x64, 4x128 or 2x128");
        if (Ho % pr) throw std::invalid_argument("conv(h2): the output height must be a multiple of the tile's rows (2 or 4)");
        if (s.nprod == 4 && (pr != 4 || bn == 32 || r.sched != ConvSched::Plain)) throw std::invalid_argument("conv(h2): four products on the plain 4x64 and 4x128 tiles");
        if (r.sched == ConvSched::Deep) throw std::invalid_argument("conv(h2): the deep schedule (1xxxx) is the stride-2 2 x 128 tile's");
        if (r.sched == ConvSched::TwoGroups && (pr != 4 || bn == 128 || r.abl || r.opt))
            throw std::invalid_argument("conv(h2): the two-group tiles are 4x32 and 4x64, without experiment variants");
        if ((r.sched == ConvSched::TwoGroups || (r.opt & 16)) && (s.cin >> 4) % 2)
            throw std::invalid_argument("conv(h2): two K groups need an even number of 16-channel slabs");
        if (s.npad % bn) throw std::invalid_argument("conv(h2): the tile width must divide the padded output width");
        p.rows = pr; p.width = bn; p.sched = r.sched;
        set_tiles(pr * kPlanTileCols, bn);
        p.xcd_gn = xcd_grid(s, r.xcd_gn, p.tiles_m, p.tiles_n, "conv(h2)");
        break;
    }
    case ConvFamily::H2S:
    case ConvFamily::H2S32:
        p.rows = kPlanTileRows; p.width = 64;
        set_tiles(128, 64);
        break;
    case ConvFamily::H2D: {
        if (r.sched == ConvSched::TwoGroups) throw std::invalid_argument("conv(h2d): the stride-2 tiles have no two-K-group form (1xxxx: the deep schedule of the 2 x 128 tile)");
        if (r.alt) throw std::invalid_argument("conv(h2d): tiles have two or four output rows");
        int pr = r.rows ? r.rows : kPlanTileRows, bn = r.width;
        if (bn == 0) {
            bn = 64;
            if (s.npad % 128 == 0 && s.cout > 64 && Ho % 2 == 0) { pr = 2; bn = 128; }
        }
        if (!(pr == 4 && (bn == 64 || bn == 128)) && !(pr == 2 && bn == 128))
            throw std::invalid_argument("conv(h2d): tile must be 4x64 (four waves), 4x128 (eight waves) or 2x128 (four waves)");
        if (s.npad % bn) throw std::invalid_argument("conv(h2d): the tile width must divide the padded output width");
        if (Ho % pr) throw std::invalid_argument("conv(h2d): the output height must be a multiple of the tile's rows");
        p.rows = pr; p.width = bn;
        set_tiles(pr * kPlanTileCols, bn);
        const bool deep = r.width ? r.sched == ConvSched::Deep : (pr == 2 && bn == 128 && s.nprod == 3 && (long)p.tiles_m * p.tiles_n <= 2L * cus);
        if (deep && s.f16) throw std::invalid_argument("conv(h2d): the deep schedule (12128) is not built for fp16 operands (one fp16 plane): fp16 x 2 operands only");
        if (deep && (pr != 2 || bn != 128 || s.nprod != 3)) throw std::invalid_argument("conv(h2d): the deep schedule is the 2 x 128 tile's, fp16 x 2 operands");
        p.sched = deep ? ConvSched::Deep : ConvSched::Plain;
        break;
    }
    case ConvFamily::H2R:
    case ConvFamily::G64: {
        if (r.abl || r.opt) throw std::invalid_argument("conv: experiment variants exist for the 3x3 / stride-1 patch kernel only");
        if (r.rows || r.sched != ConvSched::Plain || (r.width && r.width != 64 && r.width != 128)) throw std::invalid_argument("conv(h2r): the tile width must be 64 or 128");
        const bool g64_ok = (s.ks == 1 || s.ks == 3) && (s.cin & 63) == 0 && (!s.csplit || (s.csplit & 63) == 0) && s.npad % 128 == 0 && s.cout > 64;
        if (r.alt || (!r.width && g64_ok)) {
            if (!g64_ok) throw std::invalid_argument("conv(g64): needs a 1 x 1 / 3 x 3 layer, input channels in multiples of 64 and more than 64 output channels");
            p.family = ConvFamily::G64;
            p.rows = r.width ? r.width : 64; p.width = 128;
            set_tiles(p.rows, 128);
        } else {
            const long tm = (long)s.N * ((hw + 127) / 128);
            const int bn = r.width ? r.width : ((s.ks == 3 && s.cin >= 16 && wide_pays(s, tm, 1.15, cus)) ? 128 : 64);
            if (bn == 128 && (s.ks != 3 || s.cin == 8)) throw std::invalid_argument("conv(h2r): 128-wide tiles are built for 3x3 layers with at least 16 input channels");
            if (s.ks == 1 && s.cin == 8) throw std::invalid_argument("conv(h2r): 1x1 layers need at least 16 input channels");
            if (s.npad % bn) throw std::invalid_argument("conv(h2r): the tile width must divide the padded output width");
            p.family = ConvFamily::H2R;
            p.rows = 128; p.width = bn;
            set_tiles(128, bn);
        }
        break;
    }
    }
    return p;
}

inline int plan_tile_code(const ConvPlan& p) {
    if (p.family == ConvFamily::W1) return 30000 + p.rows * 1000 + p.width;
    if (p.family != ConvFamily::H2) return 0;
    return (p.side_by_side ? 3 : p.rows) * 1000 + p.width + (p.sched == ConvSched::TwoGroups ? 20000 : 0);
}

[[noreturn]] inline void plan_not_built(const ConvPlan& p, int nprod) {
    throw std::logic_error("conv: no kernel for plan family " + std::to_string((int)p.family) + ", tile " + std::to_string(p.rows) + " x " + std::to_string(p.width) +
                           (p.side_by_side ? " side by side" : "") + ", schedule " + std::to_string((int)p.sched) + ", " + std::to_string(nprod) + " products");
}

inline int head_rows(int B, int tiles_x, int hh, int cus) {
    return (long)B * tiles_x * ((hh + 31) / 32) >= cus ? 32 : ((long)B * tiles_x * ((hh + 15) / 16) >= cus ? 16 : 8);
}

}
```

### wacv23_tsnet_amd/csrc/engine.cpp

```cpp
#include <hip/hip_runtime.h>

#include <algorithm>
#include <cmath>
#include <cstdio>
#include <cstdlib>
#include <cstring>
#include <map>
#include <memory>
#include <stdexcept>
#include <string>
#include <vector>

#include "../../include/tsnet_abi.h"
#include "conv_plan.hpp"
#include "kernels.hpp"
#include "lmfit.hpp"
#include "face_adapt.hpp"
#include "flow_warp.hpp"
#include "frames.hpp"
#include "paste.hpp"
#include "head_conv.hpp"
#include "norm_elementwise.hpp"
#include "pack_weights.hpp"
#include "postproc.hpp"
// ... 88 lines not shown
        HIP_TRY(hipEventSynchronize(b));
        float t = 0.f;
        HIP_TRY(hipEventElapsedTime(&t, a, b));
        return t;
    }
};

struct SideJoin {
    hipStream_t side, main; hipEvent_t ev; bool done = false;
    ~SideJoin() { if (!done && side && hipEventRecord(ev, side) == hipSuccess) (void)hipStreamWaitEvent(main, ev, 0); }
};

struct TimeScope {
    Ctx& c;
    TimeScope(Ctx& c_, int cls) : c(c_) { if (c.timing) c.timing->begin(cls, c.stream); }
    ~TimeScope() { if (c.timing) { try { c.timing->end(c.stream); } catch (...) {} } }
};

inline void check_launch(const char* what) {
    hipError_t e = hipGetLastError();
    if (e != hipSuccess) throw std::runtime_error(std::string(what) + " launch failed: " + hipGetErrorString(e));
}

inline int ew_grid(size_t total, int block = 256) {
    size_t g = (total + block - 1) / block;
    if (g > 256 * 8) g = 256 * 8;
    if (g < 1) g = 1;
    return (int)g;
}

void launch_finalize_impl(const double* part, float* alpha, float* beta, int N, int C, int S, int HW, hipStream_t s);
inline void launch_finalize(const double* part, float* alpha, float* beta, int N, int C, int S, int HW, hipStream_t s) { launch_finalize_impl(part, alpha, beta, N, C, S, HW, s); }

inline int pack_grid(int hw) {
    int g = (hw + 255) / 256;
    if (g > 128) g = 128;
    return g < 1 ? 1 : g;
}
struct ConvLayer {
    std::string name;
    std::string wparam, bparam;
    int cin_real = 0, cin_pad = 0, cout = 0, ks = 1, stride = 1, pad = 0, reflect = 0;
    int cin_total = 0, cin_off = 0;
    int kpad = 0, npad = 0;
    int form = 0;
    size_t w_off = 0, b_off = 0;
    const unsigned short* wq = nullptr;
    const float* w_unscale = nullptr;
    const float* bias = nullptr;
};

struct DevBufs {
    std::vector<void*> p;
    template <typename T> T* alloc(size_t bytes) { void* q = nullptr; HIP_TRY(hipMalloc(&q, bytes)); p.push_back(q); return static_cast<T*>(q); }
    ~DevBufs() { for (void* q : p) (void)hipFree(q); }
    DevBufs() = default;
    DevBufs(const DevBufs&) = delete;
    DevBufs& operator=(const DevBufs&) = delete;
};

inline size_t stat_part_doubles(size_t N, size_t tpi, size_t Cout) { return N * tpi * Cout * 2; }
constexpr int KPAD_ALIGN = 32;

inline int conv_kpad(int ks, int cin_pad) { return round_up(ks * ks * cin_pad, KPAD_ALIGN); }
inline int conv_kpad_w1(int cin_pad) { return round_up(12 * cin_pad, KPAD_ALIGN); }
inline int conv_npad(int cout) { return cout >= 128 ? round_up(cout, 128) : round_up(cout, 64); }
inline int conv_cin_pad(int cin) { return cin <= 8 ? 8 : round_up(cin, 16); }

struct ConvCall {
    const float* x = nullptr; const float* x2 = nullptr;
    int csplit = 0, x2_nmod = 1;
    const float* alpha = nullptr; const float* beta = nullptr; int relu = 0;
    float bound = 0.f;
    const unsigned* in_amax = nullptr; float bound_add = 0.f;
    int N = 0, H = 0, W = 0;
    float* y = nullptr;
    const float* addend = nullptr; int add_nmod = 1;
    double* stat_part = nullptr; mutable int stat_S = 0;
    float* fin_alpha = nullptr; float* fin_beta = nullptr; int* fin_counter = nullptr;
    unsigned* amax_out = nullptr;
    int x_bf16 = 0, y_bf16 = 0;
    int nprod = 3;
    int tclass = TSNET_T_CONV;
};

inline int h2_scale_log2(float bound, int lim = 24) {
    if (!(bound > 0.f) || !std::isfinite(bound)) throw ArgError("conv: the operand bound must be positive and finite");
    int e = 0;
    (void)std::frexp(bound, &e);
    int sa = 15 - e;
    if (sa > lim) sa = lim;
    if (sa < -lim) sa = -lim;
    return sa;
}

void run_conv(Ctx& ctx, const ConvLayer& L, const ConvCall& c, ConvRequest req = {}) {
    const bool bf16 = c.nprod == 1, f16 = c.nprod == TSNET_NPROD_F16;
    if (!L.wq) throw ArgError("conv: layer has no packed weights");
    if (c.alpha && !c.beta) throw ArgError("conv: alpha without beta");
    if ((c.x_bf16 || c.y_bf16) && !bf16) throw ArgError("conv: bf16 storage goes with bf16 operands");
    if (c.x_bf16 && c.x2) throw ArgError("conv: bf16 storage of a concatenated input is not built");
    if (c.x2 && c.csplit == 0) throw ArgError("conv: a second tensor needs a channel split");
#ifdef TSNET_TOOLS
    req.chunk_cap = g_tools_knob[0];
#endif
    ConvShape sh;
    sh.ks = L.ks; sh.stride = L.stride; sh.pad = L.pad; sh.reflect = L.reflect; sh.cin = L.cin_pad; sh.cout = L.cout; sh.npad = L.npad; sh.kpad = L.kpad;
    sh.form = L.form; sh.N = c.N; sh.H = c.H; sh.W = c.W; sh.csplit = c.x2 ? c.csplit : 0; sh.x2_nmod = c.x2_nmod > 0 ? c.x2_nmod : 1;
    sh.transform = c.alpha != nullptr; sh.nprod = f16 ? 1 : c.nprod; sh.f16 = f16; sh.fin_counter = c.stat_part && c.fin_counter;
    ConvPlan p;
    try { p = plan_conv(sh, req, ctx.cus); } catch (const std::invalid_argument& e) { throw ArgError(e.what()); }
    ConvArgs g{};
    g.x = c.x; g.x2 = c.x2; g.in_alpha = c.alpha; g.in_beta = c.alpha ? c.beta : nullptr; g.in_relu = c.relu;
    const int sa = (bf16 || c.in_amax) ? 0 : h2_scale_log2(L.form == 1 ? 2.f * c.bound : c.bound, f16 ? 64 : 24);
    g.in_scale = std::ldexp(1.0f, sa); g.in_unscale = std::ldexp(1.0f, -sa);
    g.in_amax = bf16 ? nullptr : c.in_amax; g.in_bound_add = c.bound_add; g.amax_out = c.amax_out;
    g.w = L.wq; g.w_unscale = bf16 ? nullptr : L.w_unscale; g.bias = L.bias; g.y = c.y;
    g.stat_part = c.stat_part; g.addend = c.addend; g.add_nmod = c.add_nmod > 0 ? c.add_nmod : 1;
    g.x_bf16 = c.x_bf16; g.y_bf16 = c.y_bf16;
    g.N = c.N; g.H = c.H; g.W = c.W; g.Cin = L.cin_pad; g.cin_log2 = ilog2(L.cin_pad);
    g.Csplit = c.x2 ? c.csplit : L.cin_pad; g.x2_nmod = sh.x2_nmod;
    g.Ho = sh.ho(); g.Wo = sh.wo();
    g.Cout = L.cout; g.Npad = L.npad; g.stride = L.stride; g.pad = L.pad; g.reflect = L.reflect;
    g.taps = L.form == 1 ? 12 : L.ks * L.ks; g.nchunks = (g.taps * g.Cin + 15) / 16; g.M = c.N * g.Ho * g.Wo;
    g.fin_alpha = c.fin_alpha; g.fin_beta = c.fin_beta; g.fin_eps = 1e-5f;
    g.tpi = p.tpi; g.tiles_m = p.tiles_m; g.tiles_n = p.tiles_n; g.fin_S = p.tpi; g.xcd_gn = p.xcd_gn;
    g.w1_chunk = p.w1_chunk; g.w1_tab2 = p.w1_tab2; g.fin_counter = p.fin ? c.fin_counter : nullptr;
    TimeScope ts(ctx, c.tclass);
    try {
        switch (p.family) {
        case ConvFamily::W1: launch_conv_w1(g, c.nprod, req.abl, ctx.stream); break;
        case ConvFamily::H2: launch_conv_h2(g, p, c.nprod, req.abl, req.opt, ctx.stream); break;
        case ConvFamily::H2S: launch_conv_h2s(g, c.nprod, ctx.stream); break;
        case ConvFamily::H2S32: launch_conv_h2s32(g, c.nprod, ctx.stream); break;
        case ConvFamily::H2D: launch_conv_h2d(g, p, c.nprod, ctx.stream); break;
        case ConvFamily::G64: launch_conv_g64(g, p, c.nprod, ctx.stream); break;
        case ConvFamily::H2R: launch_conv_h2r(g, p, c.nprod, ctx.stream); break;
        }
    } catch (const std::invalid_argument& e) { throw ArgError(e.what()); }
    ++g_launch_counters[p.family == ConvFamily::G64 || p.family == ConvFamily::H2R ? 1 : 0];
    if (c.tclass == TSNET_T_CONV_RES && plan_tile_code(p)) g_launch_counters[3] = plan_tile_code(p);
    check_launch("conv");
    c.stat_S = !c.stat_part ? 0 : (g.fin_counter ? -1 : g.tpi);
}

void run_stats(Ctx& ctx, const float* x, int N, int HW, int C, double* part, float* alpha, float* beta) {
    if (C & 3) throw ArgError("instnorm: C must be a multiple of 4");
    TimeScope ts(ctx, TSNET_T_STATS);
    const int cq = C / 4, cols = cq < 256 ? cq : 256, R = 256 / cols;
    int S = (HW + R * 8 - 1) / (R * 8);
    if (S > 64) S = 64;
    if (S < 1) S = 1;
    const int rps = (HW + S - 1) / S;
    S = (HW + rps - 1) / rps;
    StatsArgs sa{x, part, HW, C, S, rps};
    hipLaunchKernelGGL(in_stats_partial_kernel, dim3(S, N, (cq + 255) / 256), dim3(256), 0, ctx.stream, sa);
    check_launch("in_stats_partial");
    launch_finalize(part, alpha, beta, N, C, S, HW, ctx.stream);
}

void launch_finalize_impl(const double* part, float* alpha, float* beta, int N, int C, int S, int HW, hipStream_t s) {
    if (S > 8) {
        hipLaunchKernelGGL(in_finalize2_kernel, dim3((C + kFin2Ch - 1) / kFin2Ch, N), dim3(256), 0, s, part, alpha, beta, C, S, HW, 1e-5f);
    } else {
        const int NC = N * C;
        hipLaunchKernelGGL(in_finalize_kernel, dim3((NC + 255) / 256), dim3(256), 0, s, part, alpha, beta, NC, C, S, HW, 1e-5f);
    }
    check_launch("in_finalize");
}

void run_add_stats(Ctx& ctx, const float* x, const int* slot, const float* add, int add_nmod, float* y, int N, int HW, int C, double* part, float* alpha, float* beta) {
    if (C & 3) throw ArgError("add_stats: C must be a multiple of 4");
    TimeScope ts(ctx, TSNET_T_STATS);
    const int cq = C / 4, cols = cq < 256 ? cq : 256, R = 256 / cols;
    int S = (HW + R * 8 - 1) / (R * 8);
    if (S > 64) S = 64;
    if (S < 1) S = 1;
    const int rps = (HW + S - 1) / S;
    S = (HW + rps - 1) / rps;
    const int nmod = add_nmod > 0 ? add_nmod : 1;
    AddStatsArgs sa{x, slot, add, y, part, HW, C, S, rps, nmod};
    hipLaunchKernelGGL(add_stats_partial_kernel, dim3(S, N, (cq + 255) / 256), dim3(256), 0, ctx.stream, sa);
    check_launch("add_stats_partial");
    launch_finalize(part, alpha, beta, N, C, S, HW, ctx.stream);
}

void run_norm_act(Ctx& ctx, const float* x, const float* alpha, const float* beta, int relu, const float* resid,
                  int N, int HW, int C, float* y) {
    if (C & 3) throw ArgError("norm_act: C must be a multiple of 4");
    TimeScope ts(ctx, TSNET_T_ELEMWISE);
    NormActArgs a{x, alpha, beta, resid, y, HW, C, relu, (size_t)N * HW * C / 4};
    if ((double)HW * C / 4 >= 4294967295.0 || N > 65535) throw ArgError("norm_act: tensor too large");
// ... 277 lines not shown
        return L;
    }
    void build_layers();
    void alloc_all(hipStream_t s);

    std::pair<float*, float*> next_ab(const Ctx& ctx) {
        if (!ctx.lane) { auto r = std::make_pair(ab[ab_rr][0], ab[ab_rr][1]); ab_rr = (ab_rr + 1) & 3; return r; }
        auto r = std::make_pair(ab_side[ab_side_rr][0], ab_side[ab_side_rr][1]); ab_side_rr ^= 1; return r;
    }
    float enc_bound() const { return (float)(cfg.enc_blocks + 1) * std::sqrt((float)P); }
    void conv(Ctx& ctx, const ConvLayer& L, ConvCall& c) { c.nprod = f16 ? TSNET_NPROD_F16 : np; run_conv(ctx, L, c); }
    void conv_stats(Ctx& ctx, const ConvLayer& L, ConvCall& c, int N, int HW, float* alpha, float* beta) {
        double* pt = ctx.lane ? part_side : part;
        c.stat_part = pt;
        c.fin_alpha = alpha; c.fin_beta = beta; c.fin_counter = ctx.lane ? fin_counter_side : fin_counter;
        conv(ctx, L, c);
        if (c.stat_S < 0) return;
        TimeScope ts(ctx, TSNET_T_STATS);
        hipLaunchKernelGGL(in_finalize2_kernel, dim3((L.cout + kFin2Ch - 1) / kFin2Ch, N), dim3(256), 0, ctx.stream, pt, alpha, beta, L.cout, c.stat_S, HW, 1e-5f);
        check_launch("in_finalize2");
    }
    void encode(Ctx& ctx, std::vector<ConvLayer>& L, const float* xin, const unsigned* xin_amax, int N, std::vector<float*>& raw, float* out_fea, int nblocks);
    void resblock(Ctx& ctx, const ConvLayer& c1, const ConvLayer& c2, float* Xs, float stream_bound, const unsigned* stream_amax, float amax_add,
                  float* y1, float* y2, int N, int hh, int ww);
    void set_sources(Ctx& ctx, const SrcIn& in, int B, hipStream_t bbox_stream = nullptr);
    void target_chain(Ctx& ctx, const TarIn& tar, int B);
    void bank_put(Ctx& ctx, int first, int count, const SrcIn& in, const float* div);
    void use_table(Ctx& ctx, int B, int Kc, const int* bank_slots);
    void forward_rest(Ctx& ctx, const TarIn& tar, float* out_rgb, float* out_flow, int B, int Kc, const int* bank_slots = nullptr);
    void forward_target(Ctx& ctx, const TarIn& tar, float* out_rgb, float* out_flow, int B) {
        target_chain(ctx, tar, B);
        forward_rest(ctx, tar, out_rgb, out_flow, B, K);
    }
};

void tsnet_engine::build_layers() {
    const tsnet_cfg& c = cfg;
    const int coords = c.addcoords ? 3 : 0;
    auto enc = [&](const std::string& net, int cin, int nblocks, std::vector<ConvLayer>& out) {
        const int cin_real = cin + coords;
        out.push_back(make_conv(net + ".model.1", cin_real, c.ngf, 7, 1, 3, 1));
        int idx = 4, ch = c.ngf;
        for (int i = 0; i < c.n_downsampling; ++i) {
            out.push_back(make_conv(net + ".model." + std::to_string(idx), ch, ch * 2, 3, 2, 1, 0));
            ch *= 2; idx += 3;
        }
        for (int i = 0; i < nblocks; ++i) {
            out.push_back(make_conv(net + ".model." + std::to_string(idx) + ".conv_block.1", ch, ch, 3, 1, 1, 1));
            out.push_back(make_conv(net + ".model." + std::to_string(idx) + ".conv_block.5", ch, ch, 3, 1, 1, 1));
            idx += 1;
        }
        return out[0].cin_pad;
    };
    cp_img = enc("img_enc", 3 + c.label_nc, c.enc_blocks, img_enc);
    cp_lbl = enc("lbl_enc", c.label_nc, 0, lbl_enc);
    const int fc = 2 * C;
    fuse_c1_src = make_conv("fuse_net.model.0.conv_block.1", fc, fc, 3, 1, 1, 1);
    fuse_c1_src.name += "[src]"; fuse_c1_src.cin_real = C; fuse_c1_src.cin_pad = conv_cin_pad(C); fuse_c1_src.cin_off = 0;
    fuse_c1_src.kpad = conv_kpad(3, fuse_c1_src.cin_pad);
    fuse_c1_tar = fuse_c1_src; fuse_c1_tar.name = "fuse_net.model.0.conv_block.1[tar]"; fuse_c1_tar.cin_off = C; fuse_c1_tar.bparam.clear();
    fuse_c2 = make_conv("fuse_net.model.0.conv_block.5", fc, fc, 3, 1, 1, 1);
    fuse_out = make_conv("fuse_net.conv", fc, fc / 2, 1, 1, 0, 0);
    dec_map = make_conv("dec.map_conv", 2 * C, C, 1, 1, 0, 0);
    int n = 0;
    for (int i = 0; i < c.n_blocks; ++i) {
        dec_res.push_back(make_conv("dec.model" + std::to_string(n) + ".0.conv_block.1", C, C, 3, 1, 1, 1));
        dec_res.push_back(make_conv("dec.model" + std::to_string(n) + ".0.conv_block.5", C, C, 3, 1, 1, 1));
        ++n;
    }
    for (int i = 0; i < c.n_downsampling; ++i) {
        const int ci = c.ngf << (c.n_downsampling - i);
        dec_up.push_back(make_conv("dec.model" + std::to_string(n) + ".2", ci, ci / 2, 3, 1, 1, 1));
        ++n;
    }
    dec_head = make_conv("dec.model" + std::to_string(n) + ".1", c.ngf, 3, 7, 1, 3, 1);
    auto to_w1 = [&](ConvLayer& L, int hh, int ww) {
        if (np == 1 || !w1_eligible(L.ks, L.stride, L.pad, L.cin_pad, hh, ww)) return;
        L.form = 1; L.kpad = conv_kpad_w1(L.cin_pad);
    };
    for (size_t i = 1 + c.n_downsampling; i < img_enc.size(); ++i) to_w1(img_enc[i], h, w);
    to_w1(fuse_c1_src, h, w); to_w1(fuse_c1_tar, h, w); to_w1(fuse_c2, h, w);
    for (auto& L : dec_res) to_w1(L, h, w);
    if (!dec_up.empty()) to_w1(dec_up[0], 2 * h, 2 * w);
    if (dec_up.size() > 1) to_w1(dec_up[1], 4 * h, 4 * w);
    for (auto& L : img_enc) all_layers.push_back(&L);
    for (auto& L : lbl_enc) all_layers.push_back(&L);
    all_layers.push_back(&fuse_c1_src); all_layers.push_back(&fuse_c1_tar);
    all_layers.push_back(&fuse_c2); all_layers.push_back(&fuse_out);
    all_layers.push_back(&dec_map);
    for (auto& L : dec_res) all_layers.push_back(&L);
    for (auto& L : dec_up) all_layers.push_back(&L);
}

void tsnet_engine::alloc_all(hipStream_t s) {
    const int planes = np == 1 ? 1 : 2;
    size_t off = 0;
    for (ConvLayer* L : all_layers) { L->b_off = off; off += (size_t)round_up(L->cout, 4); }
    dec_head.b_off = off; off += 4;
    off = (off + 63) / 64 * 64;
    const size_t head_off = off;
    off += (size_t)49 * cfg.ngf * 4 + 64;
    off = (off + 63) / 64 * 64;
    const size_t tab_off = off;
    off += round_up((int)all_layers.size() + 1, 64);
    off = (off + 63) / 64 * 64;
    const size_t head_planes_off = off;
    if (cfg.ngf % 16 == 0) off += head_mfma_table_halves(cfg.ngf) / 2;
    off = (off + 63) / 64 * 64;
    const size_t planes_off = off;
    size_t o16 = 0;
    for (ConvLayer* L : all_layers) { L->w_off = o16; o16 += (size_t)planes * L->kpad * L->npad; o16 = (o16 + 127) / 128 * 128; }
    off += (o16 + 1) / 2;
    wpack_floats = off;
    HIP_TRY(hipMalloc((void**)&wpack, wpack_floats * sizeof(float)));
    HIP_TRY(hipMemsetAsync(wpack, 0, wpack_floats * sizeof(float), s));
    size_t max_w = 0;
    for (ConvLayer* L : all_layers) max_w = std::max(max_w, (size_t)L->cout * L->cin_total * L->ks * (L->form == 1 ? 4 : L->ks));
    max_w = std::max(max_w, (size_t)3 * cfg.ngf * 49);
    float* stage = nullptr;
    HIP_TRY(hipMalloc((void**)&stage, max_w * sizeof(float)));
    unsigned short* planes_base = reinterpret_cast<unsigned short*>(wpack + planes_off);
    for (size_t i = 0; i < all_layers.size(); ++i) {
        ConvLayer* L = all_layers[i];
        const Param& pw = params[pindex[L->wparam]];
        std::vector<float> wino;
        if (L->form == 1) wino = winograd_x_filters(pw.host);
        const std::vector<float>& wsrc = L->form == 1 ? wino : pw.host;
        float mx = 0.f;
        for (float v : wsrc) { const float av = std::fabs(v); if (av > mx) mx = av; }
        if (!std::isfinite(mx)) throw WeightError("parameter '" + L->wparam + "' holds a non-finite value");
        const int sw = ((np != 1 || f16) && mx > 0.f) ? h2_scale_log2(mx) : 0;
        const float unscale = std::ldexp(1.0f, -sw);
        HIP_TRY(hipMemcpyAsync(stage, wsrc.data(), wsrc.size() * sizeof(float), hipMemcpyHostToDevice, s));
        HIP_TRY(hipMemcpyAsync(wpack + tab_off + i, &unscale, sizeof(float), hipMemcpyHostToDevice, s));
        pack_layer(stage, *L, planes_base + L->w_off, f16 ? -1 : planes, std::ldexp(1.0f, sw), s);
        if (!L->bparam.empty()) {
            const Param& pb = params[pindex[L->bparam]];
            HIP_TRY(hipMemcpyAsync(wpack + L->b_off, pb.host.data(), pb.host.size() * sizeof(float), hipMemcpyHostToDevice, s));
        }
        HIP_TRY(hipStreamSynchronize(s));
        L->wq = planes_base + L->w_off;
        L->w_unscale = (np == 1 && !f16) ? nullptr : wpack + tab_off + i;
        L->bias = L->bparam.empty() ? nullptr : wpack + L->b_off;
    }
    {
        const Param& pw = params[pindex[dec_head.wparam]];
        const Param& pb = params[pindex[dec_head.bparam]];
        HIP_TRY(hipMemcpyAsync(stage, pw.host.data(), pw.host.size() * sizeof(float), hipMemcpyHostToDevice, s));
        HIP_TRY(hipMemcpyAsync(wpack + dec_head.b_off, pb.host.data(), pb.host.size() * sizeof(float), hipMemcpyHostToDevice, s));
        head_w = wpack + head_off;
        head_bias = wpack + dec_head.b_off;
        hipLaunchKernelGGL(pack_head_weights_kernel, dim3(64), dim3(256), 0, s, stage, head_w, cfg.ngf);
        check_launch("pack_head_weights");
        if (cfg.ngf % 16 == 0) {
            float mx = 0.f;
            for (float v : pw.host) { const float av = std::fabs(v); if (av > mx) mx = av; }
            if (!std::isfinite(mx)) throw WeightError("parameter '" + dec_head.wparam + "' holds a non-finite value");
            const int sw = mx > 0.f ? h2_scale_log2(mx) : 0;
            const float unscale = std::ldexp(1.0f, -sw);
            const size_t slot = tab_off + all_layers.size();
            HIP_TRY(hipMemcpyAsync(wpack + slot, &unscale, sizeof(float), hipMemcpyHostToDevice, s));
            head_wq = reinterpret_cast<unsigned short*>(wpack + head_planes_off);
            head_wq_unscale = wpack + slot;
            pack_head_mfma(stage, cfg.ngf, std::ldexp(1.0f, sw), head_wq, s);
            check_launch("pack_head_mfma");
        }
        HIP_TRY(hipStreamSynchronize(s));
// ... 165 lines not shown

void tsnet_engine::target_chain(Ctx& ctx, const TarIn& tar, int B) {
    cur_B = B;
    const int H = cfg.height, W = cfg.width;
    {
        TimeScope ts(ctx, TSNET_T_PACK);
        PackArgs p{};
        p.coords = cfg.addcoords ? d_coords : nullptr;
        p.out = x_lbl; p.S = 1; p.B = B; p.H = H; p.W = W; p.L = cfg.label_nc; p.nimg = 0; p.Cp = cp_lbl;
        p.amax_out = amax_tar();
        run_pack_any(ctx, p, (size_t)3 * Bmax, tar.u8, nullptr, &tar.lbl, &tar.bbox, nullptr, tbox, 0);
    }
    encode(ctx, lbl_enc, x_lbl, amax_tar(), B, raw_lbl, tar_fea, 0);
    run_l2norm_split(ctx, tar_fea, reinterpret_cast<unsigned short*>(that), B, P, C);
    ConvCall t; t.x = tar_fea; t.bound = std::sqrt((float)P); t.N = B; t.H = h; t.W = w; t.y = FT;
    conv(ctx, fuse_c1_tar, t);
}

void tsnet_engine::use_table(Ctx& ctx, int B, int Kc, const int* bank_slots) {
    std::vector<int> t((size_t)Kc * B);
    for (int s = 0; s < Kc; ++s)
        for (int b = 0; b < B; ++b) t[s * B + b] = bank_slots ? bank_slots[s * B + b] : cached_shared ? s : s * B + b;
    if (t.size() <= slot_tab_host.size() && std::equal(t.begin(), t.end(), slot_tab_host.begin())) return;
    slot_tab_host.clear();
    run_slot_fill(ctx.stream, slot_tab, t.data(), (int)t.size());
    slot_tab_host = std::move(t);
}

void tsnet_engine::forward_rest(Ctx& ctx, const TarIn& tar, float* out_rgb, float* out_flow, int B, int Kc, const int* bank_slots) {
    cur_B = B;
    const float* tar_bbox = tar.u8 ? tbox : static_cast<const float*>(tar.bbox);
    const int K = Kc;
    const int H = cfg.height, W = cfg.width, NB = K * B;
    use_table(ctx, B, K, bank_slots);
    const int* slot = slot_tab;
    const bool fork = side_stream && !ctx.timing && ctx.lane == 0;
    Ctx cside(side_stream, cus, nullptr, 1);
    Ctx& cx = fork ? cside : ctx;
    SideJoin join2{fork ? side_stream : nullptr, ctx.stream, ev_join2};
    if (fork) {
        HIP_TRY(hipEventRecord(ev_fork2, ctx.stream));
        HIP_TRY(hipStreamWaitEvent(side_stream, ev_fork2, 0));
    }
    FlowArgs fa{};
    fa.tq = reinterpret_cast<const unsigned short*>(that); fa.sq = reinterpret_cast<const unsigned short*>(shat); fa.tar_bbox = tar_bbox;
    fa.src_bbox = bbox_copy;
    fa.gx = d_gx; fa.gy = d_gy; fa.flow = flow;
    fa.part = reinterpret_cast<unsigned long long*>(flow_part); fa.cnt = flow_cnt;
    fa.B = B; fa.P = P; fa.C = C; fa.h = h; fa.w = w; fa.H = H; fa.W = W; fa.sy = H / h; fa.sx = W / w;
    run_flow(cx, fa, NB, slot);
    if (out_flow)
        HIP_TRY(hipMemcpyAsync(out_flow, flow, (size_t)NB * P * 2 * sizeof(float), hipMemcpyDeviceToDevice, cx.stream));
    run_warp(cx, X, slot, flow, pg, B, K, h, w, C);
    if (fork) HIP_TRY(hipEventRecord(ev_join2, side_stream));

    const float sqP = std::sqrt((float)P);
    {
        auto s1 = next_ab(ctx);
        auto s2 = next_ab(ctx);
        run_add_stats(ctx, F1s, slot, FT, B, F1, NB, P, 2 * C, part, s1.first, s1.second);
        ConvCall b; b.x = F1; b.alpha = s1.first; b.beta = s1.second; b.relu = 1; b.bound = sqP;
        b.N = NB; b.H = h; b.W = w; b.y = F2;
        conv_stats(ctx, fuse_c2, b, NB, P, s2.first, s2.second);
        run_fuse_tail(ctx, FuseTailArgs{X, tar_fea, F2, s2.first, s2.second, zbar, slot, B, K, P, C});
        ConvCall c; c.x = zbar; c.bound = enc_bound() + sqP; c.N = B; c.H = h; c.W = w; c.y = sg;
        c.amax_out = amax_sg();
        conv(ctx, fuse_out, c);
    }

    if (fork) HIP_TRY(hipStreamWaitEvent(ctx.stream, ev_join2, 0));
    join2.done = true;
    {
        ConvCall a; a.x = pg; a.x2 = sg; a.csplit = C; a.x2_nmod = B; a.N = B; a.H = h; a.W = w; a.y = D;
        a.in_amax = amax_sg(); a.bound_add = enc_bound();
        a.amax_out = amax_dec();
        conv(ctx, dec_map, a);
    }
    for (int i = 0; i < cfg.n_blocks; ++i)
        resblock(ctx, dec_res[2 * i], dec_res[2 * i + 1], D, 0.f, amax_dec(), (float)i * sqP, DY1, DY2, B, h, w);
    const float* cur = D; const float* cal = nullptr; const float* cbe = nullptr;
    int hh = h, ww = w, cc = C;
    for (int i = 0; i < cfg.n_downsampling; ++i) {
        const float in_bound = std::sqrt((float)(hh * ww));
        run_upsample(ctx, cur, cal, cbe, cal ? 1 : 0, B, hh, ww, cc, U[i], st16 && i > 0, st16);
        hh *= 2; ww *= 2;
        cc /= 2;
        auto st = next_ab(ctx);
        ConvCall a; a.x = U[i]; a.bound = in_bound; a.N = B; a.H = hh; a.W = ww; a.y = R[i];
        a.x_bf16 = st16; a.y_bf16 = st16;
        if (!cal) { a.in_amax = amax_dec(); a.bound_add = (float)cfg.n_blocks * sqP; }
        conv_stats(ctx, dec_up[i], a, B, hh * ww, st.first, st.second);
        cur = R[i]; cal = st.first; cbe = st.second;
    }
    {
        TimeScope ts(ctx, TSNET_T_CONV);
        HeadArgs ha{};
        ha.x = cur; ha.alpha = cal; ha.beta = cbe; ha.w = head_w; ha.bias = head_bias; ha.y = out_rgb;
        ha.N = B; ha.H = hh; ha.W = ww; ha.C = cc; ha.x_bf16 = st16 && cfg.n_downsampling > 0;
        ha.composite = cfg.pose_composite; ha.fore_x0 = 64; ha.fore_x1 = 192;
        for (int c = 0; c < 3; ++c) ha.bg[c] = (-cfg.pose_mean[c]) / 255.0f;
        launch_head(ha, hh, ww, B, ctx.stream, ctx.cus, 0, head_wq, head_wq_unscale);
    }
    last_B = B; last_SB = bank ? 1 : cached_B; last_shared = cached_shared; last_bank = bank;
    HIP_TRY(hipEventRecord(ev_done, ctx.stream));
}

#define API_BEGIN(h)                        \
    if (!(h)) return TSNET_ERR_ARG;         \
    try {
#define API_END(h)                                                              \
    } catch (const ArgError& e) { (h)->err = e.what(); return TSNET_ERR_ARG; }   \
      catch (const WeightError& e) { (h)->err = e.what(); return TSNET_ERR_WEIGHT; } \
      catch (const std::bad_alloc&) { (h)->err = "out of host memory"; return TSNET_ERR_NOMEM; } \
      catch (const std::exception& e) { (h)->err = e.what(); return TSNET_ERR_HIP; } \
    return TSNET_OK;

extern "C" {

int tsnet_abi_version(void) { return TSNET_ABI_VERSION; }

int tsnet_create(const tsnet_cfg* cfg, tsnet_handle* out) {
    if (!cfg || !out) { g_create_error = "null argument"; return TSNET_ERR_ARG; }
    *out = nullptr;
    auto bad = [&](const char* m) { g_create_error = m; return TSNET_ERR_ARG; };
    if (cfg->n_source < 1 || cfg->n_source > TSNET_MAX_SOURCES) return bad("n_source must be in 1..8");
    if (cfg->label_nc < 1) return bad("label_nc must be >= 1");
    if (cfg->n_downsampling < 1 || cfg->n_downsampling > 5) return bad("n_downsampling must be in 1..5");
    if (cfg->ngf < 8 || (cfg->ngf & (cfg->ngf - 1))) return bad("ngf must be a power of two >= 8");
    if (cfg->n_blocks < 0 || cfg->enc_blocks < 0) return bad("block counts must be >= 0");
    const int ds = 1 << cfg->n_downsampling;
    if (cfg->height < ds * 2 || cfg->width < ds * 2 || cfg->height % ds || cfg->width % ds)
        return bad("height/width must be multiples of 2^n_downsampling (and at least twice that)");
    if (cfg->max_batch < 1) return bad("max_batch must be >= 1");
    if (cfg->pose_composite && (cfg->height != 256 || cfg->width != 256))
        return bad("pose composite is defined for 256x256 frames only (TSNet_pose.py:277-280)");
    if (cfg->operand_mode < 0 || cfg->operand_mode > 3) return bad("operand_mode must be 0 (fp32-class), 1 (bf16 operands), 2 (bf16 operands + bf16 storage) or 3 (fp16 operands)");
    try {
        tsnet_engine* e = new tsnet_engine();
        e->cfg = *cfg;
        e->K = cfg->n_source; e->Bmax = cfg->max_batch;
        for (int s = 0; s < TSNET_MAX_SOURCES; ++s) e->src_div[s] = 255.0f;
        e->C = cfg->ngf << cfg->n_downsampling;
        e->h = cfg->height / ds; e->w = cfg->width / ds; e->P = e->h * e->w;
        e->np = cfg->operand_mode != 0 ? 1 : 3;
        e->st16 = cfg->operand_mode == 2;
        e->f16 = cfg->operand_mode == 3;
        e->build_layers();
        *out = e;
    } catch (const std::exception& ex) { g_create_error = ex.what(); return TSNET_ERR_NOMEM; }
    return TSNET_OK;
}

const char* tsnet_last_error(tsnet_handle h) { return h ? h->err.c_str() : g_create_error.c_str(); }

int tsnet_num_params(tsnet_handle h) { return h ? (int)h->params.size() : TSNET_ERR_ARG; }

int tsnet_param_info(tsnet_handle h, int index, const char** name, int64_t shape_out[4], int* rank) {
    API_BEGIN(h)
    if (index < 0 || index >= (int)h->params.size()) throw ArgError("param index out of range");
    const auto& p = h->params[index];
    if (name) *name = p.name.c_str();
    if (rank) *rank = (int)p.shape.size();
    if (shape_out) for (size_t i = 0; i < 4; ++i) shape_out[i] = i < p.shape.size() ? p.shape[i] : 1;
    API_END(h)
}

int tsnet_load_weights(tsnet_handle h, const char* name, const float* data, const int64_t* shape, int rank) {
    API_BEGIN(h)
    if (h->finalized) throw ArgError("load_weights after finalize");
    if (!name || !data || !shape) throw ArgError("null argument");
    auto it = h->pindex.find(name);
    if (it == h->pindex.end()) throw WeightError(std::string("unknown parameter '") + name + "'");
// ... 314 lines not shown
    for (int i = 0; i < c.n_downsampling; ++i) {
        const double sp = P * (double)(1 << (2 * (i + 1))), ci = C / (1 << i);
        dec += sp * (ci / 2) * ci * 9;
    }
    dec += H * W * 3 * c.ngf * 49;
    const double corr = K * P * P * C + K * P * P * 2;
    return B * (K * enc(3 + c.label_nc + coords, c.enc_blocks) + enc(c.label_nc + coords, 0) + K * fuse + dec + corr);
}

int tsnet_timing_enable(tsnet_handle h, int on) {
    API_BEGIN(h)
    h->timing.on = on != 0;
    API_END(h)
}

int tsnet_timing_read(tsnet_handle h, double ms_out[TSNET_TIMING_CLASSES], int64_t launches_out[TSNET_TIMING_CLASSES], int reset) {
    API_BEGIN(h)
    h->timing.collect();
    for (int i = 0; i < TSNET_TIMING_CLASSES; ++i) {
        if (ms_out) ms_out[i] = h->timing.ms[i];
        if (launches_out) launches_out[i] = h->timing.launches[i];
        if (reset) { h->timing.ms[i] = 0; h->timing.launches[i] = 0; }
    }
    API_END(h)
}

const char* tsnet_op_last_error(void) { return g_op_error.c_str(); }

#define OP_BEGIN try {
#define OP_END                                                                   \
    } catch (const ArgError& e) { g_op_error = e.what(); return TSNET_ERR_ARG; }  \
      catch (const std::exception& e) { g_op_error = e.what(); return TSNET_ERR_HIP; } \
    return TSNET_OK;

namespace {
struct OpLayer {
    ConvLayer L;
    DevBufs mem;
    float* wd = nullptr; float* bd = nullptr; float* un = nullptr; unsigned short* wq = nullptr;
    OpLayer(const float* w_oihw, const float* bias, int Cin, int Cout, int ks, int stride, int pad, int reflect, int nprod, hipStream_t s, int form = 0) {
        L.name = "op"; L.cin_real = Cin; L.cin_pad = conv_cin_pad(Cin); L.cin_total = Cin; L.cout = Cout; L.ks = ks; L.stride = stride; L.pad = pad;
        L.reflect = reflect; L.form = form; L.kpad = form == 1 ? conv_kpad_w1(L.cin_pad) : conv_kpad(ks, L.cin_pad); L.npad = conv_npad(Cout);
        if (L.cin_pad != Cin) throw ArgError("conv2d op: Cin must be 8 or a multiple of 16 (pad channels with zeros)");
        if (form == 1 && (ks != 3 || stride != 1 || pad != 1)) throw ArgError("conv2d op: the Winograd form is for 3 x 3 / stride 1 / pad 1");
        size_t wn = (size_t)Cout * Cin * ks * ks;
        std::vector<float> hw(wn);
        HIP_TRY(hipMemcpy(hw.data(), w_oihw, wn * sizeof(float), hipMemcpyDefault));
        if (form == 1) { hw = winograd_x_filters(hw); wn = hw.size(); }
        float mx = 0.f;
        for (float v : hw) mx = std::max(mx, std::fabs(v));
        const bool f16 = nprod == TSNET_NPROD_F16;
        const int planes = (nprod == 1 || f16) ? 1 : 2;
        const int sw = (nprod != 1 && mx > 0.f) ? h2_scale_log2(mx) : 0;
        wd = mem.alloc<float>(wn * sizeof(float));
        wq = mem.alloc<unsigned short>((size_t)L.kpad * L.npad * 2 * planes);
        un = mem.alloc<float>(sizeof(float));
        HIP_TRY(hipMemcpy(wd, hw.data(), wn * sizeof(float), hipMemcpyHostToDevice));
        const float unscale = std::ldexp(1.0f, -sw);
        HIP_TRY(hipMemcpy(un, &unscale, sizeof(float), hipMemcpyHostToDevice));
        pack_layer(wd, L, wq, f16 ? -1 : planes, std::ldexp(1.0f, sw), s);
        if (bias) {
            bd = mem.alloc<float>(Cout * sizeof(float));
            HIP_TRY(hipMemcpy(bd, bias, Cout * sizeof(float), hipMemcpyDefault));
        }
        L.wq = wq; L.w_unscale = nprod == 1 ? nullptr : un; L.bias = bd;
    }
    OpLayer(const OpLayer&) = delete;
    OpLayer& operator=(const OpLayer&) = delete;
};
}

int tsnet_op_conv2d(const float* x, int N, int H, int W, int Cin, const float* w_oihw, const float* bias, int Cout,
                    int ksize, int stride, int pad, int pad_mode, const float* in_alpha, const float* in_beta, int in_relu,
                    float bound, int nprod, int kernel, int tile, float* y, void* stream) {
    OP_BEGIN
    if (!x || !w_oihw || !y) throw ArgError("null tensor");
    if (nprod != 1 && nprod != 3 && nprod != 4 && nprod != TSNET_NPROD_F16) throw ArgError("conv2d op: nprod must be 1 (bf16 operands), 16 (fp16 operands: one fp16 plane), 3 or 4 products");
    hipStream_t s = (hipStream_t)stream;
    Ctx ctx(s, current_device_cus());
    ConvRequest req;
    try { req = decode_tile_code(kernel, tile); } catch (const std::invalid_argument& e) { throw ArgError(e.what()); }
    OpLayer op(w_oihw, bias, Cin, Cout, ksize, stride, pad, pad_mode, nprod, s, kernel == 3 ? 1 : 0);
    ConvCall c; c.x = x; c.alpha = in_alpha; c.beta = in_beta; c.relu = in_relu; c.bound = bound; c.N = N; c.H = H; c.W = W; c.y = y; c.nprod = nprod;
    run_conv(ctx, op.L, c, req);
    HIP_TRY(hipStreamSynchronize(s));
    OP_END
}

int tsnet_op_conv2d_cat(const float* x, const float* x2, int N, int H, int W, int C1, int C2, int x2_nmod, const float* w_oihw, const float* bias, int Cout,
                        int ksize, int stride, int pad, int pad_mode, float bound, int nprod, float* y, void* stream) {
    OP_BEGIN
    if (!x || !x2 || !w_oihw || !y) throw ArgError("null tensor");
    hipStream_t s = (hipStream_t)stream;
    Ctx ctx(s, current_device_cus());
    OpLayer op(w_oihw, bias, C1 + C2, Cout, ksize, stride, pad, pad_mode, nprod, s);
    ConvCall c; c.x = x; c.x2 = x2; c.csplit = C1; c.x2_nmod = x2_nmod; c.bound = bound; c.N = N; c.H = H; c.W = W; c.y = y; c.nprod = nprod;
    run_conv(ctx, op.L, c);
    HIP_TRY(hipStreamSynchronize(s));
    OP_END
}

int tsnet_op_head(const float* x, int N, int H, int W, int C, const float* in_alpha, const float* in_beta, const float* w_oihw, const float* bias,
                  int composite, const float* bg, float* y, void* stream) {
    OP_BEGIN
    if (!x || !w_oihw || !bias || !y) throw ArgError("null tensor");
    if (C < 4 || (C & 3)) throw ArgError("head op: C must be a multiple of 4");
    if (in_alpha && !in_beta) throw ArgError("head op: alpha without beta");
    HeadRequest hr;
    try { hr = decode_head_code(composite); } catch (const std::invalid_argument& e) { throw ArgError(e.what()); }
    hipStream_t s = (hipStream_t)stream;
    const size_t wn = (size_t)3 * C * 49;
    DevBufs mem;
    float* wd = mem.alloc<float>(wn * sizeof(float));
    float* tab = mem.alloc<float>(((size_t)49 * C * 4 + 64) * sizeof(float));
    float* bd = mem.alloc<float>(4 * sizeof(float));
    HIP_TRY(hipMemsetAsync(tab, 0, ((size_t)49 * C * 4 + 64) * sizeof(float), s));
    HIP_TRY(hipMemcpy(wd, w_oihw, wn * sizeof(float), hipMemcpyDefault));
    HIP_TRY(hipMemcpy(bd, bias, 3 * sizeof(float), hipMemcpyDefault));
    hipLaunchKernelGGL(pack_head_weights_kernel, dim3(64), dim3(256), 0, s, wd, tab, C);
    check_launch("pack_head_weights");
    HeadArgs ha{};
    ha.x = x; ha.alpha = in_alpha; ha.beta = in_alpha ? in_beta : nullptr; ha.w = tab; ha.bias = bd; ha.y = y;
    ha.N = N; ha.H = H; ha.W = W; ha.C = C;
    ha.composite = hr.composite; ha.fore_x0 = 64; ha.fore_x1 = 192;
    for (int c = 0; c < 3; ++c) ha.bg[c] = bg ? bg[c] : 0.f;
    unsigned short* wq = nullptr; float* un = nullptr;
    if (C % 16 == 0 && in_alpha) {
        std::vector<float> hw(wn);
        HIP_TRY(hipMemcpy(hw.data(), w_oihw, wn * sizeof(float), hipMemcpyDefault));
        float mx = 0.f;
        for (float v : hw) mx = std::max(mx, std::fabs(v));
        const int sw = mx > 0.f ? h2_scale_log2(mx) : 0;
        const float unscale = std::ldexp(1.0f, -sw);
        wq = mem.alloc<unsigned short>(head_mfma_table_halves(C) * sizeof(unsigned short));
        un = mem.alloc<float>(sizeof(float));
        HIP_TRY(hipMemcpy(un, &unscale, sizeof(float), hipMemcpyHostToDevice));
        pack_head_mfma(wd, C, std::ldexp(1.0f, sw), wq, s);
        check_launch("pack_head_mfma");
    }
    launch_head(ha, H, W, N, s, current_device_cus(), hr.rows, wq, un);
    HIP_TRY(hipStreamSynchronize(s));
    OP_END
}

int tsnet_op_instnorm_stats(const float* x, int N, int HW, int C, float* alpha, float* beta, void* stream) {
    OP_BEGIN
    if (!x || !alpha || !beta) throw ArgError("null tensor");
    Ctx ctx((hipStream_t)stream, current_device_cus());
    DevBufs mem;
    double* part = mem.alloc<double>((size_t)N * 64 * C * 2 * sizeof(double));
    run_stats(ctx, x, N, HW, C, part, alpha, beta);
    HIP_TRY(hipStreamSynchronize(ctx.stream));
    OP_END
}

int tsnet_op_norm_act(const float* x, const float* alpha, const float* beta, int relu, const float* resid,
                      int N, int HW, int C, float* y, void* stream) {
    OP_BEGIN
    if (!x || !y) throw ArgError("null tensor");
    Ctx ctx((hipStream_t)stream, current_device_cus());
    run_norm_act(ctx, x, alpha, beta, relu, resid, N, HW, C, y);
    OP_END
}

int tsnet_op_upsample2x(const float* x, const float* alpha, const float* beta, int relu, int N, int H, int W, int C, float* y, void* stream) {
    OP_BEGIN
// ... 780 lines not shown
```

### wacv23_tsnet_amd/csrc/norm_elementwise.hpp

```cpp
#pragma once
#include <hip/hip_runtime.h>

#include "conv_common.hpp"

namespace tsnet {

struct StatsArgs {
    const float* x;
    double* part;
    int HW, C, S, rows_per_split;
};

__global__ __launch_bounds__(256) void in_stats_partial_kernel(StatsArgs a) {
    __shared__ double red[256 * 8];
    const int cq_total = a.C >> 2;
    const int cols = cq_total < 256 ? cq_total : 256;
    const int R = 256 / cols;
    const int tid = threadIdx.x;
    const int cq = tid % cols + blockIdx.z * 256;
    const int rg = tid / cols;
    const int n = blockIdx.y, s = blockIdx.x;
    const int r0 = s * a.rows_per_split;
    int r1 = r0 + a.rows_per_split;
    if (r1 > a.HW) r1 = a.HW;
// ... 170 lines not shown
            }
            v.x = __builtin_fmaf(v.x, al.x, be.x);
            v.y = __builtin_fmaf(v.y, al.y, be.y);
            v.z = __builtin_fmaf(v.z, al.z, be.z);
            v.w = __builtin_fmaf(v.w, al.w, be.w);
        }
        if (a.relu) {
            v.x = v.x > 0.f ? v.x : 0.f; v.y = v.y > 0.f ? v.y : 0.f;
            v.z = v.z > 0.f ? v.z : 0.f; v.w = v.w > 0.f ? v.w : 0.f;
        }
        if (a.resid) {
            const float4 r = reinterpret_cast<const float4*>(a.resid)[i];
            v.x = r.x + v.x; v.y = r.y + v.y; v.z = r.z + v.z; v.w = r.w + v.w;
        }
        reinterpret_cast<float4*>(a.y)[i] = v;
    }
}

struct FuseTailArgs {
    const float* src_fea;
    const float* tar_fea;
    const float* y2;
    const float* alpha;
    const float* beta;
    float* zbar;
    const int* slot;
    int B, K, P, C1;
};

__global__ __launch_bounds__(256) void fuse_resid_mean_kernel(FuseTailArgs a) {
    const int C = 2 * a.C1;
    const int c4n = C >> 2;
    const size_t total = (size_t)a.B * a.P * c4n;
    const size_t stride = (size_t)gridDim.x * blockDim.x;
    for (size_t i = (size_t)blockIdx.x * blockDim.x + threadIdx.x; i < total; i += stride) {
        const int c = (int)(i % c4n) * 4;
        const size_t bp = i / c4n;
        const int b = (int)(bp / a.P);
        const int p = (int)(bp - (size_t)b * a.P);
        float4 acc = make_float4(0.f, 0.f, 0.f, 0.f);
        for (int s = 0; s < a.K; ++s) {
            const int n = s * a.B + b;
            float4 xr;
            if (c < a.C1) xr = *reinterpret_cast<const float4*>(a.src_fea + ((size_t)a.slot[n] * a.P + p) * a.C1 + c);
            else          xr = *reinterpret_cast<const float4*>(a.tar_fea + ((size_t)b * a.P + p) * a.C1 + (c - a.C1));
            const float4 y = *reinterpret_cast<const float4*>(a.y2 + ((size_t)n * a.P + p) * C + c);
            const float4 al = *reinterpret_cast<const float4*>(a.alpha + (size_t)n * C + c);
            const float4 be = *reinterpret_cast<const float4*>(a.beta + (size_t)n * C + c);
            acc.x += xr.x + __builtin_fmaf(y.x, al.x, be.x);
            acc.y += xr.y + __builtin_fmaf(y.y, al.y, be.y);
            acc.z += xr.z + __builtin_fmaf(y.z, al.z, be.z);
            acc.w += xr.w + __builtin_fmaf(y.w, al.w, be.w);
        }
        const float kf = (float)a.K;
        acc.x /= kf; acc.y /= kf; acc.z /= kf; acc.w /= kf;
        *reinterpret_cast<float4*>(a.zbar + ((size_t)b * a.P + p) * C + c) = acc;
    }
}

constexpr int kSlotFill = 64;
struct SlotFillArgs { int* dst; int n; int v[kSlotFill]; };
__global__ __launch_bounds__(64) void slot_fill_kernel(SlotFillArgs a) {
    const int i = threadIdx.x;
    if (i < a.n) a.dst[i] = a.v[i];
}

struct UpsampleArgs {
    const float* x;
    const float* alpha;
    const float* beta;
    float* y;
    int N, H, W, C, relu;
    int x_bf16, y_bf16;
};

__device__ __forceinline__ float4 ld4_f32_or_bf16(const float* base, size_t elem, bool b16) {
    if (!b16) return *reinterpret_cast<const float4*>(base + elem);
    const uint2 p = *reinterpret_cast<const uint2*>(reinterpret_cast<const unsigned short*>(base) + elem);
    return make_float4(__builtin_bit_cast(float, p.x << 16), __builtin_bit_cast(float, p.x & 0xFFFF0000u),
                       __builtin_bit_cast(float, p.y << 16), __builtin_bit_cast(float, p.y & 0xFFFF0000u));
}

__device__ __forceinline__ float4 na4(float4 v, const float4& al, const float4& be, bool norm, bool relu) {
    if (norm) {
        v.x = __builtin_fmaf(v.x, al.x, be.x); v.y = __builtin_fmaf(v.y, al.y, be.y);
        v.z = __builtin_fmaf(v.z, al.z, be.z); v.w = __builtin_fmaf(v.w, al.w, be.w);
    }
    if (relu) {
        v.x = v.x > 0.f ? v.x : 0.f; v.y = v.y > 0.f ? v.y : 0.f;
        v.z = v.z > 0.f ? v.z : 0.f; v.w = v.w > 0.f ? v.w : 0.f;
    }
    return v;
}

__global__ __launch_bounds__(256) void upsample2x_kernel(UpsampleArgs a) {
    const unsigned c4n = (unsigned)a.C >> 2;
    const int Ho = 2 * a.H, Wo = 2 * a.W;
    const int oy = blockIdx.y, n = blockIdx.z;
    const unsigned row4 = (unsigned)Wo * c4n;
    for (unsigned j = blockIdx.x * 256u + threadIdx.x; j < row4; j += gridDim.x * 256u) {
        const int ox = (int)(j / c4n);
        const int c = (int)(j - (unsigned)ox * c4n) * 4;
        const size_t i = ((size_t)n * Ho + oy) * row4 + j;
        float sy = (oy + 0.5f) * 0.5f - 0.5f; if (sy < 0.f) sy = 0.f;
        float sx = (ox + 0.5f) * 0.5f - 0.5f; if (sx < 0.f) sx = 0.f;
        const int y0 = (int)sy, x0 = (int)sx;
        const int y1 = y0 + (y0 < a.H - 1 ? 1 : 0), x1 = x0 + (x0 < a.W - 1 ? 1 : 0);
        const float wy1 = sy - y0, wy0 = 1.f - wy1, wx1 = sx - x0, wx0 = 1.f - wx1;
        const bool norm = a.alpha != nullptr;
        float4 al = make_float4(1.f, 1.f, 1.f, 1.f), be = make_float4(0.f, 0.f, 0.f, 0.f);
        if (norm) {
            al = *reinterpret_cast<const float4*>(a.alpha + (size_t)n * a.C + c);
            be = *reinterpret_cast<const float4*>(a.beta + (size_t)n * a.C + c);
        }
        const size_t base = ((size_t)n * a.H * a.W) * a.C + c;
        const bool xb = a.x_bf16 != 0;
        const float4 v00 = na4(ld4_f32_or_bf16(a.x, base + ((size_t)y0 * a.W + x0) * a.C, xb), al, be, norm, a.relu);
        const float4 v01 = na4(ld4_f32_or_bf16(a.x, base + ((size_t)y0 * a.W + x1) * a.C, xb), al, be, norm, a.relu);
        const float4 v10 = na4(ld4_f32_or_bf16(a.x, base + ((size_t)y1 * a.W + x0) * a.C, xb), al, be, norm, a.relu);
        const float4 v11 = na4(ld4_f32_or_bf16(a.x, base + ((size_t)y1 * a.W + x1) * a.C, xb), al, be, norm, a.relu);
        float4 o;
        o.x = wy0 * (wx0 * v00.x + wx1 * v01.x) + wy1 * (wx0 * v10.x + wx1 * v11.x);
        o.y = wy0 * (wx0 * v00.y + wx1 * v01.y) + wy1 * (wx0 * v10.y + wx1 * v11.y);
        o.z = wy0 * (wx0 * v00.z + wx1 * v01.z) + wy1 * (wx0 * v10.z + wx1 * v11.z);
        o.w = wy0 * (wx0 * v00.w + wx1 * v01.w) + wy1 * (wx0 * v10.w + wx1 * v11.w);
        if (a.y_bf16) {
            uint2 q;
            q.x = TSNET_CVT_PK_BF16(o.x, o.y);
            q.y = TSNET_CVT_PK_BF16(o.z, o.w);
            reinterpret_cast<uint2*>(a.y)[i] = q;
        } else {
            reinterpret_cast<float4*>(a.y)[i] = o;
        }
    }
}

__global__ void bf16_widen_kernel(const unsigned short* __restrict__ x, float* __restrict__ y, size_t n) {
    for (size_t i = (size_t)blockIdx.x * blockDim.x + threadIdx.x; i < n; i += (size_t)gridDim.x * blockDim.x)
        y[i] = __builtin_bit_cast(float, (unsigned)x[i] << 16);
}

struct PackArgs {
    const float* img[8];
    const float* lbl[8];
    const float* coords;
    float* out;
    int S, B, H, W, L, nimg, Cp;
    float img_div[8];
    unsigned* amax_out;
};

__global__ __launch_bounds__(256) void pack_input_kernel(PackArgs a) {
    const size_t HW = (size_t)a.H * a.W;
    const int creal = a.nimg + a.L + (a.coords ? 3 : 0);
    const int n = blockIdx.y;
    const int s = n / a.B, b = n - s * a.B;
    const float* const img_b = a.nimg ? a.img[s] + (size_t)b * a.nimg * HW : a.lbl[s];
    const float* const lbl_b = a.lbl[s] + (size_t)b * a.L * HW;
    const float* const dummy = a.lbl[s];
    const float div = a.img_div[s];
    float vmax = 0.f;
    for (size_t pix = (size_t)blockIdx.x * blockDim.x + threadIdx.x; pix < HW; pix += (size_t)gridDim.x * blockDim.x) {
        float* o = a.out + ((size_t)n * HW + pix) * a.Cp;
        for (int c0 = 0; c0 < a.Cp; c0 += 8) {
            float v[8];
#pragma unroll
            for (int e = 0; e < 8; ++e) {
                const int c = c0 + e;
                const bool is_img = c < a.nimg, is_lbl = !is_img && c < a.nimg + a.L, is_crd = !is_img && !is_lbl && c < creal;
                const float* p = is_img ? img_b + (size_t)c * HW : (is_lbl ? lbl_b + (size_t)(c - a.nimg) * HW : (is_crd ? a.coords + (c - a.nimg - a.L) : dummy));
                const size_t idx = is_crd ? pix * 3 : ((is_img || is_lbl) ? pix : 0);
                const float t = p[idx];
                v[e] = (is_img || is_lbl || is_crd) ? t : 0.f;
            }
#pragma unroll
            for (int e = 0; e < 8; ++e) {
                if (c0 + e < a.nimg) v[e] = v[e] / div;
                vmax = __builtin_fmaxf(vmax, __builtin_fabsf(v[e]));
            }
            *reinterpret_cast<float4*>(o + c0) = make_float4(v[0], v[1], v[2], v[3]);
            *reinterpret_cast<float4*>(o + c0 + 4) = make_float4(v[4], v[5], v[6], v[7]);
        }
    }
    if (a.amax_out) tsnet_publish_amax(a.amax_out + n, vmax);
}

struct PackU8Args {
    const unsigned char* img[8];
    const unsigned char* lbl[8];
    const unsigned char* bbox[8];
    const float* coords;
    float* out;
    float* bbox_out;
    size_t bbox_sstride;
    int S, B, H, W, L, nimg, Cp;
    float img_div[8];
    float mean[3];
    unsigned* amax_out;
};

constexpr int kPackU8Px = 4;

__device__ __forceinline__ unsigned pack_u8_ld4(const unsigned char* plane, size_t pix, int cnt) {
    const unsigned char* p = plane + pix;
    if (cnt == kPackU8Px && (reinterpret_cast<uintptr_t>(p) & 3u) == 0) return *reinterpret_cast<const unsigned*>(p);
    unsigned v = 0;
#pragma unroll
    for (int i = 0; i < kPackU8Px; ++i)
// ... 74 lines not shown
```

Before: 817.2 frames/s.

## Fuse bilinear x2 upsample and input norm into decoder 3x3 convolution

Adds a patch-kernel variant that loads the half-resolution activation into LDS, applies the instance-norm affine and ReLU, then bilinearly upsamples and splits into fp16 pairs while staging the conv input. This removes the separate upsample kernel and its full-resolution intermediate write and read. The decoder uses it when the plan accepts it (fp32 storage, three products, reflection, 4-row tiles). In exchange it adds LDS for the low-res buffers, extra per-thread index setup and a new pipeline schedule inside the conv loop.

```diff
diff --git a/include/tsnet_abi.h b/include/tsnet_abi.h
--- a/include/tsnet_abi.h
+++ b/include/tsnet_abi.h
@@ -101,6 +101,10 @@
                     const float* w_oihw, const float* bias, int Cout, int ksize, int stride, int pad, int pad_mode,
                     const float* in_alpha, const float* in_beta, int in_relu, float bound, int nprod, int kernel, int tile,
                     float* y, void* stream);
+int tsnet_op_upconv2d(const float* x, int N, int H, int W, int Cin,
+                      const float* w_oihw, const float* bias, int Cout, int ksize, int stride, int pad, int pad_mode,
+                      const float* in_alpha, const float* in_beta, int in_relu, float bound, int nprod, int kernel, int tile,
+                      float* y, void* stream);
 int tsnet_op_conv2d_cat(const float* x, const float* x2, int N, int H, int W, int C1, int C2, int x2_nmod,
                         const float* w_oihw, const float* bias, int Cout, int ksize, int stride, int pad, int pad_mode,
                         float bound, int nprod, float* y, void* stream);
diff --git a/wacv23_tsnet_amd/_lib.py b/wacv23_tsnet_amd/_lib.py
--- a/wacv23_tsnet_amd/_lib.py
+++ b/wacv23_tsnet_amd/_lib.py
@@ -27,6 +27,7 @@
     "tsnet_paste_frames",
     "tsnet_prepare_frames_boxes", "tsnet_prepare_frames_boxes_u8", "tsnet_paste_frames_boxes",
     "tsnet_face_labels_boxes", "tsnet_face_labels_boxes_u8",
+    "tsnet_op_upconv2d",
 )
 
 
@@ -140,6 +141,8 @@
     if hasattr(lib, "tsnet_face_labels_boxes"):
         for fn in (lib.tsnet_face_labels_boxes, lib.tsnet_face_labels_boxes_u8):
             fn.argtypes = [_vp, _vp, C.c_int, _vp, _vp, _vp, C.c_int, C.c_int, _vp, C.c_longlong, C.c_int, C.c_int, _vp, _vp, _vp]
+    if hasattr(lib, "tsnet_op_upconv2d"):
+        lib.tsnet_op_upconv2d.argtypes = lib.tsnet_op_conv2d.argtypes
     return lib
 
 
diff --git a/wacv23_tsnet_amd/csrc/conv_common.hpp b/wacv23_tsnet_amd/csrc/conv_common.hpp
--- a/wacv23_tsnet_amd/csrc/conv_common.hpp
+++ b/wacv23_tsnet_amd/csrc/conv_common.hpp
@@ -248,6 +248,22 @@
     }
 }
 
+__device__ __forceinline__ void up2_source(int o, int n, int& i0, int& i1, float& w0, float& w1) {
+    float s = (o + 0.5f) * 0.5f - 0.5f; if (s < 0.f) s = 0.f;
+    i0 = (int)s;
+    i1 = i0 + (i0 < n - 1 ? 1 : 0);
+    w1 = s - i0; w0 = 1.f - w1;
+}
+__device__ __forceinline__ float up2_tap(float v, float al, float be, bool norm, bool relu) {
+    if (norm) v = __builtin_fmaf(v, al, be);
+    if (relu) v = v > 0.f ? v : 0.f;
+    return v;
+}
+__device__ __forceinline__ float up2_lerp(float a, float b, float w0, float w1) { return w0 * a + w1 * b; }
+__device__ __forceinline__ float up2_blend(float v00, float v01, float v10, float v11, float wx0, float wx1, float wy0, float wy1) {
+    return up2_lerp(up2_lerp(v00, v01, wx0, wx1), up2_lerp(v10, v11, wx0, wx1), wy0, wy1);
+}
+
 template <int BN, int WARPS_M, int WARPS_N, int MT, int NTL, int STAT_WAVE = 0, typename MOf>
 __device__ __forceinline__ void conv_epilogue(const ConvArgs& a, f32x16 (&tot)[MT][NTL], unsigned char* smem_raw, int tid, int wave, int n0,
                                               size_t stat_tile, MOf m_of, const bool active = true) {
diff --git a/wacv23_tsnet_amd/csrc/conv_h2.hpp b/wacv23_tsnet_amd/csrc/conv_h2.hpp
--- a/wacv23_tsnet_amd/csrc/conv_h2.hpp
+++ b/wacv23_tsnet_amd/csrc/conv_h2.hpp
@@ -3,7 +3,7 @@
 
 namespace tsnet {
 
-template <int PR, int BN, int WARPS_M, int WARPS_N, int NPROD, bool AFFINE, int HABL = 0, int OPT = 0>
+template <int PR, int BN, int WARPS_M, int WARPS_N, int NPROD, bool AFFINE, int HABL = 0, int OPT = 0, bool UP2 = false>
 __device__ __forceinline__ void h2_tile(const ConvArgs& a, unsigned char* smem_raw, const int tile_m, const int n0) {
     constexpr int BM = PR * kPatchCols;
     constexpr int NW = WARPS_M * WARPS_N;
@@ -28,7 +28,11 @@
     constexpr int PLANE_P = 2 * REGION, PATCH_BYTES = NPL * PLANE_P;
     constexpr int OFF_SINK = 2 * 2 * PLANE_P;
     constexpr int GROUP_BYTES = OFF_SINK + 2048;
-    constexpr int OFF_TAB = KG * GROUP_BYTES;
+    constexpr int LPC = kPatchCols / 2 + 2, LPP = (PR / 2 + 2) * LPC;
+    constexpr int LQ = LPP * 16, LBUF = 4 * LQ;
+    constexpr int OFF_LOW = KG * GROUP_BYTES;
+    constexpr int OFF_TAB = OFF_LOW + (UP2 ? 2 * LBUF : 0);
+    static_assert(!UP2 || (PR == 4 && NPROD == 3 && KG == 1 && !DEEP && !ZPAD_KEEP && HABL == 0), "fused upsample: fp16 x 2 operands, four-row tiles, plain schedule, reflection");
 
     const int tid = threadIdx.x;
     const int lane = tid & 63;
@@ -49,7 +53,7 @@
 
     const size_t planew = (size_t)((a.nchunks + 1) / 2 * 2) * a.Npad * 16;
     const bool xb16 = NPROD == 1 && a.x_bf16;
-    const tsnet_brsrc_t rsx = tsnet_make_brsrc(a.x, (unsigned)((size_t)a.N * a.H * a.W * a.Cin * (xb16 ? 2 : 4)));
+    const tsnet_brsrc_t rsx = tsnet_make_brsrc(a.x, (unsigned)((size_t)a.N * (UP2 ? (a.H >> 1) * (a.W >> 1) : a.H * a.W) * a.Cin * (xb16 ? 2 : 4)));
     tsnet_brsrc_t rsw[NPL];
 #pragma unroll
     for (int p = 0; p < NPL; ++p) rsw[p] = tsnet_make_brsrc(a.w + p * planew, (unsigned)(planew * 2));
@@ -75,11 +79,44 @@
         vP[r] = ok ? (unsigned)(((img * a.H * a.W + pix) * a.Cin + oct * 8) * 4) : kOOB;
         vM[r] = ok ? 1.f : 0.f;
     }
+    unsigned vL = kOOB;
+    int oL = -1;
+    const int octL = tid < LPP ? 0 : 1;
+    if (UP2) {
+        const int lp = tid < LPP ? tid : tid - LPP;
+        const int ly = (oy0 >> 1) - 1 + lp / LPC, lx = (ox0 >> 1) - 1 + lp % LPC;
+        const int Hl = a.H >> 1, Wl = a.W >> 1;
+        if (tid < 2 * LPP) {
+            oL = (2 * octL * LPP + lp) * 16;
+            if (ly >= 0 && ly < Hl && lx >= 0 && lx < Wl) vL = (unsigned)(((img * Hl * Wl + ly * Wl + lx) * a.Cin + octL * 8) * 4);
+        }
+    }
+    int uA = 0, uDx = 0, uDst = 0;
+    float uWx = 0.f, uWyA = 0.f, uWyB = 0.f;
+    bool uSelA = false;
+    if (UP2) {
+        const int octU = tid >> 7;
+        int idx = tid & 127;
+        idx = idx < 3 * PC ? idx : idx - 64;
+        const int j = idx / PC, pc = idx - j * PC;
+        auto refl = [](int i, int n) { i = i < 0 ? -i : i; return i >= n ? 2 * (n - 1) - i : i; };
+        const int ix = refl(ox0 - 1 + pc, a.W), iyA = refl(oy0 - 1 + 2 * j, a.H), iyB = refl(oy0 + 2 * j, a.H);
+        int x0, x1, r0, r1, a0, a1;
+        float w0;
+        up2_source(ix, a.W >> 1, x0, x1, w0, uWx);
+        up2_source(iyB, a.H >> 1, r0, r1, w0, uWyB);
+        up2_source(iyA, a.H >> 1, a0, a1, w0, uWyA);
+        uSelA = a0 != r0;
+        uA = (2 * octU * LPP + (r0 - ((oy0 >> 1) - 1)) * LPC + x0 - ((ox0 >> 1) - 1)) * 16;
+        uDx = (x1 - x0) * 16;
+        uDst = octU * REGION + (2 * j * PC + pc) * 16;
+    }
     float* tab = reinterpret_cast<float*>(smem_raw + OFF_TAB);
     if (AFFINE) {
+        const float ts = UP2 ? 1.f : in_scale;
         for (int c = tid; c < a.Cin; c += 256 * KG) {
-            tab[c] = a.in_alpha[(size_t)img * a.Cin + c] * in_scale;
-            tab[a.Cin + c] = a.in_beta[(size_t)img * a.Cin + c] * in_scale;
+            tab[c] = a.in_alpha[(size_t)img * a.Cin + c] * ts;
+            tab[a.Cin + c] = a.in_beta[(size_t)img * a.Cin + c] * ts;
         }
         __syncthreads();
     }
@@ -108,6 +145,48 @@
             *reinterpret_cast<F4*>(dst) = Hh;
             *reinterpret_cast<F4*>(dst + (b < PBLK ? PLANE_P : 1024)) = Ll;
         }
+    };
+
+    F4 sl[2][2];
+    auto low_load = [&](int cn, int set) __attribute__((always_inline)) {
+#pragma unroll
+        for (int q = 0; q < 2; ++q) sl[set][q] = TSNET_BUF_LOAD16(rsx, vL, (unsigned)(cn * 64 + q * 16));
+    };
+    auto low_store = [&](int cn, int set, int lb) __attribute__((always_inline)) {
+        const float* ta = tab + (cn < ncc ? cn * 16 : 0) + octL * 8;
+        F4 t[2];
+#pragma unroll
+        for (int q = 0; q < 2; ++q) {
+            F4 al = sl[set][q], be = sl[set][q];
+            if (AFFINE) { al = *reinterpret_cast<const F4*>(ta + q * 4); be = *reinterpret_cast<const F4*>(ta + a.Cin + q * 4); }
+#pragma unroll
+            for (int e = 0; e < 4; ++e) t[q].v[e] = up2_tap(sl[set][q].v[e], al.v[e], be.v[e], AFFINE, AFFINE && a.in_relu);
+        }
+        unsigned char* dst = smem_raw + (oL >= 0 ? OFF_LOW + lb * LBUF + oL : OFF_SINK + lane * 16);
+        *reinterpret_cast<F4*>(dst) = t[0];
+        *reinterpret_cast<F4*>(dst + (oL >= 0 ? LQ : 0)) = t[1];
+    };
+    auto up_pair = [&](int lb, int par, int h) __attribute__((always_inline)) {
+        const unsigned char* p = smem_raw + OFF_LOW + lb * LBUF + h * LQ + uA;
+        const F4 v00 = *reinterpret_cast<const F4*>(p), v01 = *reinterpret_cast<const F4*>(p + uDx);
+        const F4 v10 = *reinterpret_cast<const F4*>(p + LPC * 16), v11 = *reinterpret_cast<const F4*>(p + LPC * 16 + uDx);
+        const float wx0 = 1.f - uWx, wa0 = 1.f - uWyA, wb0 = 1.f - uWyB;
+        float oa[4], ob[4];
+#pragma unroll
+        for (int e = 0; e < 4; ++e) {
+            const float h0 = up2_lerp(v00.v[e], v01.v[e], wx0, uWx), h1 = up2_lerp(v10.v[e], v11.v[e], wx0, uWx);
+            oa[e] = up2_lerp(uSelA ? h1 : h0, h1, wa0, uWyA);
+            ob[e] = up2_lerp(h0, h1, wb0, uWyB);
+        }
+        unsigned ha[2], la[2], hb[2], lb2[2];
+        TSNET_SPLIT_2PAIRS_SCALED(oa[0], oa[1], oa[2], oa[3], in_scale, ha[0], la[0], ha[1], la[1]);
+        TSNET_SPLIT_2PAIRS_SCALED(ob[0], ob[1], ob[2], ob[3], in_scale, hb[0], lb2[0], hb[1], lb2[1]);
+        unsigned char* dst = gbase + par * PATCH_BYTES + uDst + h * 8;
+        struct alignas(8) U2 { unsigned v[2]; };
+        *reinterpret_cast<U2*>(dst) = U2{{ha[0], ha[1]}};
+        *reinterpret_cast<U2*>(dst + PLANE_P) = U2{{la[0], la[1]}};
+        *reinterpret_cast<U2*>(dst + PC * 16) = U2{{hb[0], hb[1]}};
+        *reinterpret_cast<U2*>(dst + PC * 16 + PLANE_P) = U2{{lb2[0], lb2[1]}};
     };
 
     const unsigned vB = (unsigned)((wn0 + li) * 32 + (lh ^ ((li >> 3) & 1)) * 16);
@@ -170,8 +249,12 @@
                 if (kx < 2 && ky == 2) load_row(MT - 1, par, kx + 1);
             }
         }
-        if (s == 0 && !(HABL & 1)) stage_load_x(cc + 1, 0);
-        if (s == (DEEP ? 1 : 3) && !(HABL & 1)) stage_load_x(cc + 1, 1);
+        if (UP2) {
+            if (s == 6) low_load(cc + 2, 0);
+        } else {
+            if (s == 0 && !(HABL & 1)) stage_load_x(cc + 1, 0);
+            if (s == (DEEP ? 1 : 3) && !(HABL & 1)) stage_load_x(cc + 1, 1);
+        }
         const int SB = (par * 9 + s) % BD;
         if (ONEP) {
             product(kx, ky, SB, 0, 0, fresh);
@@ -181,8 +264,14 @@
             product(kx, ky, SB, 0, NPL - 1, false);
             product(kx, ky, SB, 0, 0, false);
         }
-        if (s == (DEEP ? 5 : 2) && !(HABL & 1)) stage_store(cc + 1, par ^ 1, 0);
-        if (s == (DEEP ? 7 : 5) && !(HABL & 1)) stage_store(cc + 1, par ^ 1, 1);
+        if (UP2) {
+            if (s == 1) up_pair(par ^ 1, par ^ 1, 0);
+            if (s == 4) up_pair(par ^ 1, par ^ 1, 1);
+            if (s == 8) low_store(cc + 2, 0, par);
+        } else {
+            if (s == (DEEP ? 5 : 2) && !(HABL & 1)) stage_store(cc + 1, par ^ 1, 0);
+            if (s == (DEEP ? 7 : 5) && !(HABL & 1)) stage_store(cc + 1, par ^ 1, 1);
+        }
         __builtin_amdgcn_sched_barrier(0);
         if (!ONE_LEVEL && last && !(HABL & 8)) {
 #pragma unroll
@@ -204,10 +293,20 @@
         wsl += KG * wB;
     };
 
-    stage_load_x(0, 0); stage_load_x(0, 1);
-#pragma unroll
-    for (int i = 0; i < BD - 1; ++i) load_b(i, 0, i);
-    stage_store(0, 0, 0); stage_store(0, 0, 1);
+    if (UP2) {
+        low_load(0, 0); low_load(1, 1);
+#pragma unroll
+        for (int i = 0; i < BD - 1; ++i) load_b(i, 0, i);
+        low_store(0, 0, 0); low_store(1, 1, 1);
+        __syncthreads();
+#pragma unroll
+        for (int h = 0; h < 2; ++h) up_pair(0, 0, h);
+    } else {
+        stage_load_x(0, 0); stage_load_x(0, 1);
+#pragma unroll
+        for (int i = 0; i < BD - 1; ++i) load_b(i, 0, i);
+        stage_store(0, 0, 0); stage_store(0, 0, 1);
+    }
     if (HABL & 2) load_b(2, 0, 2);
     if (HABL & 4) {
         __syncthreads();
@@ -265,7 +364,9 @@
                                                  [&](int l) { return m_img + (oy0 + (l >> 5)) * a.Wo + ox0 + (l & 31); }, kg == 0);
 }
 
-constexpr int h2_lds_bytes(int PR, int Cin, int KG = 1) { return KG * (2 * 2 * 2 * (((PR + 2) * (kPatchCols + 2) + 31) / 32) * 512 + 2048) + 2 * Cin * 4; }
+constexpr int h2_lds_bytes(int PR, int Cin, int KG = 1, bool up2 = false) {
+    return KG * (2 * 2 * 2 * (((PR + 2) * (kPatchCols + 2) + 31) / 32) * 512 + 2048) + (up2 ? 2 * (PR / 2 + 2) * (kPatchCols / 2 + 2) * 64 : 0) + 2 * Cin * 4;
+}
 
 template <int PR, int BN, int WARPS_M, int WARPS_N, int NPROD, int OPT>
 constexpr int h2_wgs_per_cu() { return (OPT & 16) ? 1 : ((BN / WARPS_N) * (PR / WARPS_M) * ((OPT & 8) ? 2 : 1) <= (one_product(NPROD) ? 128 : 64) ? ((OPT & 64) ? 4 : 3) : 2); }
@@ -277,6 +378,15 @@
     int tile_m, tile_n;
     tile_of_block(blockIdx.x, a.tiles_m, a.tiles_n, a.xcd_gn, tile_m, tile_n);
     h2_tile<PR, BN, WARPS_M, WARPS_N, NPROD, AFFINE, HABL, OPT>(a, smem_raw, tile_m, tile_n * BN);
+}
+
+template <int PR, int BN, int WARPS_M, int WARPS_N, int NPROD, bool AFFINE>
+__global__ __launch_bounds__(256, (h2_wgs_per_cu<PR, BN, WARPS_M, WARPS_N, NPROD, 0>()))
+void conv_h2u_kernel(ConvArgs a) {
+    HIP_DYNAMIC_SHARED(__attribute__((aligned(16))) unsigned char, smem_raw)
+    int tile_m, tile_n;
+    tile_of_block(blockIdx.x, a.tiles_m, a.tiles_n, a.xcd_gn, tile_m, tile_n);
+    h2_tile<PR, BN, WARPS_M, WARPS_N, NPROD, AFFINE, 0, 0, true>(a, smem_raw, tile_m, tile_n * BN);
 }
 
 template <int NPROD>
diff --git a/wacv23_tsnet_amd/csrc/conv_h2_launch.cpp b/wacv23_tsnet_amd/csrc/conv_h2_launch.cpp
--- a/wacv23_tsnet_amd/csrc/conv_h2_launch.cpp
+++ b/wacv23_tsnet_amd/csrc/conv_h2_launch.cpp
@@ -40,6 +40,13 @@
     else go_h2_k<PR, BN, WM, WN, NPROD, true, HABL, OPT | 1>(a, lds, 256 * KG, s);
 }
 
+template <int BN>
+void go_h2u(const ConvArgs& a, hipStream_t s) {
+    const size_t lds = (size_t)h2_lds_bytes(4, a.Cin, 1, true);
+    if (a.in_alpha) launch_tiles(conv_h2u_kernel<4, BN, 2, 2, 3, true>, 256, lds, a, s);
+    else launch_tiles(conv_h2u_kernel<4, BN, 2, 2, 3, false>, 256, lds, a, s);
+}
+
 template <int NPROD>
 void go_h2_shape(const ConvArgs& a, const ConvPlan& p, hipStream_t s) {
     const int pr = p.rows, bn = p.width;
@@ -62,6 +69,11 @@
 
 void launch_conv_h2(const ConvArgs& a, const ConvPlan& p, int nprod, int abl, int opt, hipStream_t s) {
     const int pr = p.rows, bn = p.width;
+    if (p.up2) {
+        if (nprod == 3 && !abl && !opt && p.sched == ConvSched::Plain && !p.side_by_side && a.reflect && pr == 4 && bn == 64) return go_h2u<64>(a, s);
+        if (nprod == 3 && !abl && !opt && p.sched == ConvSched::Plain && !p.side_by_side && a.reflect && pr == 4 && bn == 128) return go_h2u<128>(a, s);
+        plan_not_built(p, nprod);
+    }
     if (p.sched == ConvSched::TwoGroups) {
         if (pr == 4 && bn == 32) return nprod == 3 ? go_h2<4, 32, 4, 1, 3, 0, 24>(a, s) : (nprod == kNprodF16 ? go_h2<4, 32, 4, 1, kNprodF16, 0, 24>(a, s) : go_h2<4, 32, 4, 1, 1, 0, 24>(a, s));
         if (pr == 4 && bn == 64) return nprod == 3 ? go_h2<4, 64, 2, 2, 3, 0, 24>(a, s) : (nprod == kNprodF16 ? go_h2<4, 64, 2, 2, kNprodF16, 0, 24>(a, s) : go_h2<4, 64, 2, 2, 1, 0, 24>(a, s));
diff --git a/wacv23_tsnet_amd/csrc/conv_plan.hpp b/wacv23_tsnet_amd/csrc/conv_plan.hpp
--- a/wacv23_tsnet_amd/csrc/conv_plan.hpp
+++ b/wacv23_tsnet_amd/csrc/conv_plan.hpp
@@ -25,6 +25,7 @@
     int nprod = 3;
     bool f16 = false;
     bool fin_counter = false;
+    bool up2 = false;
     int ho() const { return (H + 2 * pad - ks) / stride + 1; }
     int wo() const { return (W + 2 * pad - ks) / stride + 1; }
 };
@@ -51,6 +52,7 @@
     int xcd_gn = 0;
     int tpi = 0, tiles_m = 0, tiles_n = 0;
     bool fin = false;
+    bool up2 = false;
 };
 
 inline ConvRequest decode_tile_code(int kernel, int tile) {
@@ -189,6 +191,8 @@
         p.family = conv_class(s, r.rows == 2 ? 2 : kPlanTileRows, r.kernel == ConvKernel::Patch);
         if (r.kernel == ConvKernel::Patch && p.family == ConvFamily::H2R) throw std::invalid_argument("conv: this layer / frame size has no patch kernel");
     }
+    if (s.up2 && (p.family != ConvFamily::H2 || !s.reflect || s.nprod != 3 || (s.H & 1) || (s.W & 1)))
+        throw std::invalid_argument("conv: a half-resolution input (fused x2 upsample) needs the 3x3 / stride-1 patch kernel, reflection padding, fp16 x 2 operands (three products) and an even frame");
     if (s.nprod != 1 && s.nprod != 3 && (s.nprod != 4 || p.family != ConvFamily::H2))
         throw std::invalid_argument("conv: 1 (bf16 operands), 16 (fp16 operands) or 3 products; four on the 3x3 / stride-1 patch kernel's plain 4x64 and 4x128 tiles");
     if (s.f16 && s.nprod != 1) throw std::invalid_argument("conv: fp16 operands (one fp16 plane) run one product");
@@ -223,6 +227,9 @@
         if ((r.sched == ConvSched::TwoGroups || (r.opt & 16)) && (s.cin >> 4) % 2)
             throw std::invalid_argument("conv(h2): two K groups need an even number of 16-channel slabs");
         if (s.npad % bn) throw std::invalid_argument("conv(h2): the tile width must divide the padded output width");
+        if (s.up2 && (pr != 4 || bn == 32 || p.side_by_side || r.sched != ConvSched::Plain || r.abl || r.opt))
+            throw std::invalid_argument("conv(h2): the fused x2 upsample is built for the plain 4x64 and 4x128 tiles");
+        p.up2 = s.up2;
         p.rows = pr; p.width = bn; p.sched = r.sched;
         set_tiles(pr * kPlanTileCols, bn);
         p.xcd_gn = xcd_grid(s, r.xcd_gn, p.tiles_m, p.tiles_n, "conv(h2)");
@@ -279,6 +286,11 @@
     return p;
 }
 
+inline bool plan_takes_up2(ConvShape s, int cus) {
+    s.up2 = true;
+    try { return plan_conv(s, ConvRequest{}, cus).up2; } catch (const std::invalid_argument&) { return false; }
+}
+
 inline int plan_tile_code(const ConvPlan& p) {
     if (p.family == ConvFamily::W1) return 30000 + p.rows * 1000 + p.width;
     if (p.family != ConvFamily::H2) return 0;
diff --git a/wacv23_tsnet_amd/csrc/engine.cpp b/wacv23_tsnet_amd/csrc/engine.cpp
--- a/wacv23_tsnet_amd/csrc/engine.cpp
+++ b/wacv23_tsnet_amd/csrc/engine.cpp
@@ -194,6 +194,7 @@
     int x_bf16 = 0, y_bf16 = 0;
     int nprod = 3;
     int tclass = TSNET_T_CONV;
+    bool up2 = false;
 };
 
 inline int h2_scale_log2(float bound, int lim = 24) {
@@ -204,6 +205,16 @@
     if (sa > lim) sa = lim;
     if (sa < -lim) sa = -lim;
     return sa;
+}
+
+ConvShape conv_shape(const ConvLayer& L, const ConvCall& c) {
+    const bool f16 = c.nprod == TSNET_NPROD_F16;
+    ConvShape sh;
+    sh.ks = L.ks; sh.stride = L.stride; sh.pad = L.pad; sh.reflect = L.reflect; sh.cin = L.cin_pad; sh.cout = L.cout; sh.npad = L.npad; sh.kpad = L.kpad;
+    sh.form = L.form; sh.N = c.N; sh.H = c.H; sh.W = c.W; sh.csplit = c.x2 ? c.csplit : 0; sh.x2_nmod = c.x2_nmod > 0 ? c.x2_nmod : 1;
+    sh.transform = c.alpha != nullptr; sh.nprod = f16 ? 1 : c.nprod; sh.f16 = f16; sh.fin_counter = c.stat_part && c.fin_counter;
+    sh.up2 = c.up2;
+    return sh;
 }
 
 void run_conv(Ctx& ctx, const ConvLayer& L, const ConvCall& c, ConvRequest req = {}) {
@@ -216,10 +227,8 @@
 #ifdef TSNET_TOOLS
     req.chunk_cap = g_tools_knob[0];
 #endif
-    ConvShape sh;
-    sh.ks = L.ks; sh.stride = L.stride; sh.pad = L.pad; sh.reflect = L.reflect; sh.cin = L.cin_pad; sh.cout = L.cout; sh.npad = L.npad; sh.kpad = L.kpad;
-    sh.form = L.form; sh.N = c.N; sh.H = c.H; sh.W = c.W; sh.csplit = c.x2 ? c.csplit : 0; sh.x2_nmod = c.x2_nmod > 0 ? c.x2_nmod : 1;
-    sh.transform = c.alpha != nullptr; sh.nprod = f16 ? 1 : c.nprod; sh.f16 = f16; sh.fin_counter = c.stat_part && c.fin_counter;
+    if (c.up2 && (c.x_bf16 || c.y_bf16 || c.in_amax)) throw ArgError("conv: the fused x2 upsample takes fp32 tensors and an a-priori operand bound");
+    const ConvShape sh = conv_shape(L, c);
     ConvPlan p;
     try { p = plan_conv(sh, req, ctx.cus); } catch (const std::invalid_argument& e) { throw ArgError(e.what()); }
     ConvArgs g{};
@@ -663,7 +672,11 @@
     to_w1(fuse_c1_src, h, w); to_w1(fuse_c1_tar, h, w); to_w1(fuse_c2, h, w);
     for (auto& L : dec_res) to_w1(L, h, w);
     if (!dec_up.empty()) to_w1(dec_up[0], 2 * h, 2 * w);
-    if (dec_up.size() > 1) to_w1(dec_up[1], 4 * h, 4 * w);
+    bool up1_w1 = true;
+#ifdef TSNET_TOOLS
+    up1_w1 = g_tools_knob[2] == 0;
+#endif
+    if (dec_up.size() > 1 && up1_w1) to_w1(dec_up[1], 4 * h, 4 * w);
     for (auto& L : img_enc) all_layers.push_back(&L);
     for (auto& L : lbl_enc) all_layers.push_back(&L);
     all_layers.push_back(&fuse_c1_src); all_layers.push_back(&fuse_c1_tar);
@@ -995,12 +1008,21 @@
     int hh = h, ww = w, cc = C;
     for (int i = 0; i < cfg.n_downsampling; ++i) {
         const float in_bound = std::sqrt((float)(hh * ww));
-        run_upsample(ctx, cur, cal, cbe, cal ? 1 : 0, B, hh, ww, cc, U[i], st16 && i > 0, st16);
+        bool fused = false;
+        if (cal && !st16) {
+            ConvCall q; q.N = B; q.H = 2 * hh; q.W = 2 * ww; q.alpha = cal; q.nprod = f16 ? TSNET_NPROD_F16 : np;
+            fused = plan_takes_up2(conv_shape(dec_up[i], q), ctx.cus);
+        }
+#ifdef TSNET_TOOLS
+        if (g_tools_knob[1]) fused = false;
+#endif
+        if (!fused) run_upsample(ctx, cur, cal, cbe, cal ? 1 : 0, B, hh, ww, cc, U[i], st16 && i > 0, st16);
         hh *= 2; ww *= 2;
         cc /= 2;
         auto st = next_ab(ctx);
         ConvCall a; a.x = U[i]; a.bound = in_bound; a.N = B; a.H = hh; a.W = ww; a.y = R[i];
         a.x_bf16 = st16; a.y_bf16 = st16;
+        if (fused) { a.x = cur; a.alpha = cal; a.beta = cbe; a.relu = 1; a.up2 = true; }
         if (!cal) { a.in_amax = amax_dec(); a.bound_add = (float)cfg.n_blocks * sqP; }
         conv_stats(ctx, dec_up[i], a, B, hh * ww, st.first, st.second);
         cur = R[i]; cal = st.first; cbe = st.second;
@@ -1481,6 +1503,35 @@
     try { req = decode_tile_code(kernel, tile); } catch (const std::invalid_argument& e) { throw ArgError(e.what()); }
     OpLayer op(w_oihw, bias, Cin, Cout, ksize, stride, pad, pad_mode, nprod, s, kernel == 3 ? 1 : 0);
     ConvCall c; c.x = x; c.alpha = in_alpha; c.beta = in_beta; c.relu = in_relu; c.bound = bound; c.N = N; c.H = H; c.W = W; c.y = y; c.nprod = nprod;
+    run_conv(ctx, op.L, c, req);
+    HIP_TRY(hipStreamSynchronize(s));
+    OP_END
+}
+
+int tsnet_op_upconv2d(const float* x, int N, int H, int W, int Cin, const float* w_oihw, const float* bias, int Cout,
+                      int ksize, int stride, int pad, int pad_mode, const float* in_alpha, const float* in_beta, int in_relu,
+                      float bound, int nprod, int kernel, int tile, float* y, void* stream) {
+    OP_BEGIN
+    if (!x || !w_oihw || !y) throw ArgError("null tensor");
+    if (ksize != 3 || stride != 1 || pad != 1 || pad_mode != 1) throw ArgError("upconv2d op: a 3 x 3 / stride-1 / pad-1 layer with reflection padding");
+    if (nprod != 3) throw ArgError("upconv2d op: fp16 x 2 operands (nprod = 3) and fp32 tensors");
+    if (kernel != 0 && kernel != 1) throw ArgError("upconv2d op: kernel 0 (fused) or 1 (upsample2x, then the convolution)");
+    if (in_alpha && !in_beta) throw ArgError("upconv2d op: alpha without beta");
+    if (N < 1 || H < 1 || W < 1 || (double)N * H * W * 4 * Cin >= 536870912.0) throw ArgError("upconv2d op: empty or too large a tensor");
+    hipStream_t s = (hipStream_t)stream;
+    Ctx ctx(s, current_device_cus());
+    ConvRequest req;
+    try { req = decode_tile_code(0, tile); } catch (const std::invalid_argument& e) { throw ArgError(e.what()); }
+    OpLayer op(w_oihw, bias, Cin, Cout, ksize, stride, pad, pad_mode, nprod, s);
+    ConvCall c; c.x = x; c.alpha = in_alpha; c.beta = in_beta; c.relu = in_alpha ? in_relu : 0; c.bound = bound; c.N = N; c.H = 2 * H; c.W = 2 * W; c.y = y; c.nprod = nprod;
+    c.up2 = true;
+    try { (void)plan_conv(conv_shape(op.L, c), req, ctx.cus); } catch (const std::invalid_argument& e) { throw ArgError(e.what()); }
+    DevBufs mem;
+    if (kernel == 1) {
+        float* up = mem.alloc<float>((size_t)N * 2 * H * 2 * W * Cin * sizeof(float));
+        run_upsample(ctx, x, in_alpha, in_alpha ? in_beta : nullptr, c.relu, N, H, W, Cin, up);
+        c.x = up; c.alpha = nullptr; c.beta = nullptr; c.relu = 0; c.up2 = false;
+    }
     run_conv(ctx, op.L, c, req);
     HIP_TRY(hipStreamSynchronize(s));
     OP_END
diff --git a/wacv23_tsnet_amd/csrc/norm_elementwise.hpp b/wacv23_tsnet_amd/csrc/norm_elementwise.hpp
--- a/wacv23_tsnet_amd/csrc/norm_elementwise.hpp
+++ b/wacv23_tsnet_amd/csrc/norm_elementwise.hpp
@@ -276,14 +276,8 @@
 }
 
 __device__ __forceinline__ float4 na4(float4 v, const float4& al, const float4& be, bool norm, bool relu) {
-    if (norm) {
-        v.x = __builtin_fmaf(v.x, al.x, be.x); v.y = __builtin_fmaf(v.y, al.y, be.y);
-        v.z = __builtin_fmaf(v.z, al.z, be.z); v.w = __builtin_fmaf(v.w, al.w, be.w);
-    }
-    if (relu) {
-        v.x = v.x > 0.f ? v.x : 0.f; v.y = v.y > 0.f ? v.y : 0.f;
-        v.z = v.z > 0.f ? v.z : 0.f; v.w = v.w > 0.f ? v.w : 0.f;
-    }
+    v.x = up2_tap(v.x, al.x, be.x, norm, relu); v.y = up2_tap(v.y, al.y, be.y, norm, relu);
+    v.z = up2_tap(v.z, al.z, be.z, norm, relu); v.w = up2_tap(v.w, al.w, be.w, norm, relu);
     return v;
 }
 
@@ -296,11 +290,10 @@
         const int ox = (int)(j / c4n);
         const int c = (int)(j - (unsigned)ox * c4n) * 4;
         const size_t i = ((size_t)n * Ho + oy) * row4 + j;
-        float sy = (oy + 0.5f) * 0.5f - 0.5f; if (sy < 0.f) sy = 0.f;
-        float sx = (ox + 0.5f) * 0.5f - 0.5f; if (sx < 0.f) sx = 0.f;
-        const int y0 = (int)sy, x0 = (int)sx;
-        const int y1 = y0 + (y0 < a.H - 1 ? 1 : 0), x1 = x0 + (x0 < a.W - 1 ? 1 : 0);
-        const float wy1 = sy - y0, wy0 = 1.f - wy1, wx1 = sx - x0, wx0 = 1.f - wx1;
+        int y0, y1, x0, x1;
+        float wy0, wy1, wx0, wx1;
+        up2_source(oy, a.H, y0, y1, wy0, wy1);
+        up2_source(ox, a.W, x0, x1, wx0, wx1);
         const bool norm = a.alpha != nullptr;
         float4 al = make_float4(1.f, 1.f, 1.f, 1.f), be = make_float4(0.f, 0.f, 0.f, 0.f);
         if (norm) {
@@ -314,10 +307,10 @@
         const float4 v10 = na4(ld4_f32_or_bf16(a.x, base + ((size_t)y1 * a.W + x0) * a.C, xb), al, be, norm, a.relu);
         const float4 v11 = na4(ld4_f32_or_bf16(a.x, base + ((size_t)y1 * a.W + x1) * a.C, xb), al, be, norm, a.relu);
         float4 o;
-        o.x = wy0 * (wx0 * v00.x + wx1 * v01.x) + wy1 * (wx0 * v10.x + wx1 * v11.x);
-        o.y = wy0 * (wx0 * v00.y + wx1 * v01.y) + wy1 * (wx0 * v10.y + wx1 * v11.y);
-        o.z = wy0 * (wx0 * v00.z + wx1 * v01.z) + wy1 * (wx0 * v10.z + wx1 * v11.z);
-        o.w = wy0 * (wx0 * v00.w + wx1 * v01.w) + wy1 * (wx0 * v10.w + wx1 * v11.w);
+        o.x = up2_blend(v00.x, v01.x, v10.x, v11.x, wx0, wx1, wy0, wy1);
+        o.y = up2_blend(v00.y, v01.y, v10.y, v11.y, wx0, wx1, wy0, wy1);
+        o.z = up2_blend(v00.z, v01.z, v10.z, v11.z, wx0, wx1, wy0, wy1);
+        o.w = up2_blend(v00.w, v01.w, v10.w, v11.w, wx0, wx1, wy0, wy1);
         if (a.y_bf16) {
             uint2 q;
             q.x = TSNET_CVT_PK_BF16(o.x, o.y);
```

After: 828.5 frames/s (median of 6 runs). 1.01x the previous value.
